# IntelLabs/coach

Measured on AMD Instinct MI355X. Metric: env-steps/sec (+ grad-updates/sec) on Atari-like Clipped-PPO, 64 vectorized envs/GPU, higher is better.
Workload: dtype f32; 1 GPU; C2: Atari-Pong-like Clipped-PPO, 64 vectorized envs/GPU, 84x84x4 uint8 obs, GAE(0.99,0.95), rollout 2048 env-steps (episodes of 32), 10 epochs x 32 minibatches of 64, fp32 conv torso x2 (value/policy), TF1-Adam; parallelism=dp1 (env vectors sharded per GPU, flat fp32 gradient all-reduce), hip_graphs=True

## Files before the change

### coach_amd/_rlx.py

```python
import ctypes
import os
import re
import subprocess
import threading

_HERE = os.path.dirname(os.path.abspath(__file__))
_ROOT = os.path.dirname(_HERE)
HEADER = os.path.join(_ROOT, "include", "rlx.h")
LIB_PATH = os.path.join(_HERE, "librlx.so")
CSRC = os.path.join(_HERE, "csrc")


class RlxUnavailable(RuntimeError):
    """librlx.so is missing or cannot be loaded; the HIP hot path cannot run."""


class RlxError(RuntimeError):
    """A librlx entry point returned a non-zero rlx_status."""


_CTYPE = {
    "int": ctypes.c_int,
    "unsigned": ctypes.c_uint,
    "unsigned int": ctypes.c_uint,
# ... 245 lines not shown

class SplitkJob(STRUCTS["rlx_splitk_job"]):
    __doc__ = STRUCTS["rlx_splitk_job"].__doc__

    def workspace_floats(self):
        return (self.M * self.N + self.N) * self.batch * self.splits if self.splits > 1 else 0


ABI_VERSION = CONSTANTS["RLX_ABI_VERSION"]
NOISY_PASSES = CONSTANTS["RLX_NOISY_PASSES"]
NOISY_MAX_LAYERS = CONSTANTS["RLX_NOISY_MAX_LAYERS"]
NOISY_PASS = {"act": 0, "online": 1, "target": 2, "online_next": 3}
assert sorted(NOISY_PASS.values()) == list(range(NOISY_PASSES)), "NOISY_PASS names every pass of RLX_NOISY_PASSES"
ADAM_TICKET_WORDS = CONSTANTS["RLX_ADAM_TICKET_WORDS"]
MAX_SPLITK_JOBS = CONSTANTS["RLX_MAX_SPLITK_JOBS"]
MAX_COLUMNS = CONSTANTS["RLX_MAX_COLUMNS"]
ACT = {None: CONSTANTS["RLX_ACT_NONE"]}
ACT.update((k[len("RLX_ACT_"):].lower(), v) for k, v in CONSTANTS.items() if k.startswith("RLX_ACT_"))


def make_columns(pairs):
    arr = (Column * len(pairs))()
    for i, (s, d) in enumerate(pairs):
        rb = (s[0].numel() if s.dim() > 1 else 1) * s.element_size()
        arr[i] = Column(s.data_ptr(), d.data_ptr(), rb)
    return arr


def splitk_reduce_jobs(jobs, stream=None, ppo_tail=None, per_tail=None):
    live = [j for j in jobs if j.splits > 1]
    s = current_stream() if stream is None else stream
    for i in range(0, len(live), MAX_SPLITK_JOBS):
        chunk = live[i:i + MAX_SPLITK_JOBS]
        arr = (SplitkJob * len(chunk))(*chunk)
        if per_tail is not None and ppo_tail is None and i + MAX_SPLITK_JOBS >= len(live):
            run = lambda a=arr, n=len(chunk), t=per_tail: lib().splitk_reduce_jobs_per_update(ctypes.byref(a), n, *t, s)
            per_tail = None
        elif ppo_tail is not None and i + MAX_SPLITK_JOBS >= len(live):
            run = lambda a=arr, n=len(chunk), t=ppo_tail: lib().splitk_reduce_jobs_ppo_tail(ctypes.byref(a), n, ctypes.byref(t), s)
            ppo_tail = None
        else:
            run = lambda a=arr, n=len(chunk): lib().splitk_reduce_jobs(ctypes.byref(a), n, s)
        _record((), run, flops=0.0)
        run()
    if ppo_tail is not None:
        lib().ppo_heads_tail(ctypes.byref(ppo_tail), s)
    if per_tail is not None:
        lib().per_update(*per_tail, s)


def conv_input_grad(dz, weights, dx, x_out, deriv, tables, B, H, W, C, KH, KW, S, Co, towers, dy_stride, w_stride,
                    dx_stride, stream=None):
    s = current_stream() if stream is None else stream
    OH, OW = (H - KH) // S + 1, (W - KW) // S + 1
    run = lambda: lib().conv_input_grad(dz, weights, dx, x_out, ACT[deriv], tables, B, H, W, C, KH, KW, S, Co, towers,
                                        dy_stride, w_stride, dx_stride, s)
    if GEMM_HOOK is not None:
        d = GemmDesc()
        d.M, d.N, d.K, d.batch = B * OH * OW, KH * KW * C, Co, towers
        _record((d,), run)
    run()


def per_update_desc(args):
    sum_t, min_t, max_t, cap, idx, err, n, alpha, eps, maxp, status = args
    d = PerUpdateDesc()
    d.sum_tree, d.min_tree, d.max_tree, d.capacity = sum_t.data_ptr(), min_t.data_ptr(), max_t.data_ptr(), int(cap)
    d.idx, d.td_errors, d.n, d.alpha, d.epsilon = idx.data_ptr(), err.data_ptr(), int(n), float(alpha), float(eps)
    d.max_priority, d.status = maxp.data_ptr(), status.data_ptr()
    return d


def conv_dw_item(x, x_tower_stride, x_is_u8, a_div, dz, dz_tower_stride, B, H, W, C, KH, KW, S, Co, towers, dw, dw_tower_stride, db,
                 db_tower_stride, workspace):
    it = ConvDwItem()
    it.x, it.x_tower_stride, it.x_is_u8, it.a_div = x.data_ptr(), x_tower_stride, int(bool(x_is_u8)), float(a_div)
    it.dz, it.dz_tower_stride = dz.data_ptr(), dz_tower_stride
    it.B, it.H, it.W, it.C, it.KH, it.KW, it.S, it.filters, it.towers = B, H, W, C, KH, KW, S, Co, towers
    it.dw, it.dw_tower_stride, it.db, it.db_tower_stride = dw.data_ptr(), dw_tower_stride, _ptr(db), db_tower_stride
    it.workspace, it.workspace_floats = workspace.data_ptr(), workspace.numel()
    return it


def conv_dw_multi(items, jobs, stream=None):
    s = current_stream() if stream is None else stream
    n = len(items)
    arr = (ConvDwItem * n)(*items)
    jarr = (SplitkJob * n)()

    def run():
        lib().conv_dw_multi(arr, jarr, n, s)
    if GEMM_HOOK is not None:
        descs = []
        for it in items:
            OH, OW = (it.H - it.KH) // it.S + 1, (it.W - it.KW) // it.S + 1
            d = GemmDesc()
            d.M, d.K = it.KH * it.KW * it.C, it.B * OH * OW
            d.N, d.batch, d.a_is_u8 = (it.towers * it.filters, 1, 1) if it.x_is_u8 else (it.filters, it.towers, 0)
            descs.append(d)
        _record(tuple(descs), run)
    run()
    for j, out in zip(jarr, jobs):
        ctypes.memmove(ctypes.byref(out), ctypes.byref(j), ctypes.sizeof(SplitkJob))


GEMM_HOOK = None
CALL_COUNT = 0


def _ptr(t):
    return None if t is None else (t.data_ptr() if hasattr(t, "data_ptr") else t)


def gemm(M, N, K, A, B, C, *, a_strides=None, a_tabs=None, a_u8=False, a_div=1.0,
         a_vec_along_k=1, a_tab_vec_ok=0, b_strides=None, ldc=None, bias=None, activation=None,
         deriv_aux=None, aux_ld=None, deriv_kind=None, accumulate=False, batch=1,
         a_batch_stride=0, b_batch_stride=0, c_batch_stride=0, bias_batch_stride=0,
         aux_batch_stride=0, workspace=None, colsum_out=None, colsum_batch_stride=0, stream=None,
         batch_inner=0, a_batch_stride2=0, b_batch_stride2=0, bias_batch_stride2=0, n_fold=0, launch=True,
         defer=None, row_heads=None, kw_min_tiles=0):
    d = GemmDesc()
    d.M, d.N, d.K, d.batch = int(M), int(N), int(K), int(batch)
    d.A, d.B, d.C = _ptr(A), _ptr(B), _ptr(C)
    if a_tabs is not None:
        d.a_row_tab, d.a_k_tab = _ptr(a_tabs[0]), _ptr(a_tabs[1])
        d.a_row_stride, d.a_k_stride = 0, 0
    else:
        rs, ks = a_strides if a_strides is not None else (K, 1)
        d.a_row_stride, d.a_k_stride = int(rs), int(ks)
    ks, ns = b_strides if b_strides is not None else (N, 1)
    d.b_k_stride, d.b_n_stride = int(ks), int(ns)
    d.a_batch_stride, d.b_batch_stride = int(a_batch_stride), int(b_batch_stride)
    d.ldc = int(N if ldc is None else ldc)
    d.c_batch_stride, d.bias_batch_stride = int(c_batch_stride), int(bias_batch_stride)
    d.bias, d.deriv_aux = _ptr(bias), _ptr(deriv_aux)
    d.aux_ld = int(N if aux_ld is None else aux_ld)
    d.aux_batch_stride = int(aux_batch_stride)
    d.workspace = _ptr(workspace)
    d.colsum_out, d.colsum_batch_stride = _ptr(colsum_out), int(colsum_batch_stride)
    d.workspace_floats = int(workspace.numel()) if workspace is not None else 0
    d.a_is_u8, d.a_div = int(bool(a_u8)), float(a_div)
    d.a_vec_along_k, d.a_tab_vec_ok = int(a_vec_along_k), int(a_tab_vec_ok)
    d.activation, d.deriv_kind = ACT[activation], ACT[deriv_kind]
    d.accumulate = int(bool(accumulate))
    d.batch_inner = int(batch_inner)
    d.a_batch_stride2, d.b_batch_stride2 = int(a_batch_stride2), int(b_batch_stride2)
    d.bias_batch_stride2 = int(bias_batch_stride2)
    d.n_fold = int(n_fold)
    d.kw_min_tiles = int(kw_min_tiles)
    if row_heads is not None:
        d._row_heads = row_heads
        d.row_heads, d.n_row_heads = ctypes.addressof(row_heads), len(row_heads)
    if not launch:
        return d
    s = current_stream() if stream is None else stream
    if defer is not None:
        run = lambda: lib().gemm_defer(ctypes.byref(d), ctypes.byref(defer), s)
    else:
        run = lambda: lib().gemm(ctypes.byref(d), s)
    _record((d,), run)
    run()


def _record(descs, run, flops=None):
    if GEMM_HOOK is not None:
        GEMM_HOOK({"descs": tuple(GemmDesc.from_buffer_copy(x) for x in descs), "run": run, "flops": flops})


def gemm_pair_or_single(desc, stream=None):
    s = current_stream() if stream is None else stream
    run = lambda: lib().gemm(ctypes.byref(desc), s)
    _record((desc,), run)
    run()

# ... 24 lines not shown
```

### coach_amd/agents/clipped_ppo_agent.py

```python
import os
import random

import numpy as np
import torch

from .. import _rlx
from ..core_types import EnvironmentSteps, RunPhase
from ..memories.episodic.episodic_rollout_buffer import DeviceEpisodicRolloutBuffer
from ..nn.networks import ClippedPPONet
from ..schedules import ConstantSchedule


from ..architectures.scheme_views import SchemeViews


class ClippedPPONetworkParameters(SchemeViews):
    def __init__(self):
        self.activation_function = 'tanh'
        self.embedder_scheme = 'Medium'
        self.middleware_scheme = 'Medium'
        self.batch_size = 64
        self.optimizer_type = 'Adam'
        self.learning_rate = 0.00025
        self.adam_optimizer_beta1 = 0.9
# ... 418 lines not shown
            if self.dist is None:
                mem.gather_next_states(rows, n, self.ds_obs_raw[:n])
                self.norm.push(self.ds_obs_raw[:n])

        def chunk_obs(c0, m):
            if self.norm is not None:
                return self.ds_obs[c0:c0 + m]
            return mem.gather_states(rows[c0:c0 + m], m, self.chunk_obs[:m])
        for c0 in range(0, 0 if recorded else n, self.chunk):
            m = min(self.chunk, n - c0)
            net.values(chunk_obs(c0, m), m, out=self.ds_value[c0:c0 + m])
        n_seq = 1 if self.ragged else mem.n_env
        self.lib.gae(self.ds_reward, self.ds_value, self.ds_done, None, n_seq, n // n_seq,
                     alg.discount, alg.gae_lambda, self.ds_adv64, self.ds_vtarget, s)
        self.lib.standardize(self.ds_adv64, n, self.ds_adv, None, self.adv_stats, s)
        for c0 in range(0, 0 if recorded else n_train, self.chunk):
            m = min(self.chunk, n_train - c0)
            if self.continuous:
                net.policy_mean_std(chunk_obs(c0, m), m, use_target=True, tag="old",
                                    out_mean=self.ds_old_probs[c0:c0 + m], out_std=self.ds_old_std[c0:c0 + m])
            else:
                net.policy_probs(chunk_obs(c0, m), m, use_target=True, tag="old",
                                 out=self.ds_old_probs[c0:c0 + m])

    def fill_advantages(self):
        n = self.memory.num_transitions()
        rows = self.memory.dataset_rows()
        if self.norm is not None and self.dist is not None:
            self.memory.gather_states(rows, n, self.ds_obs_raw[:n])
            self.norm.push_shared(self.ds_obs_raw[:n], self.dist)
        n_train = min(n, self.ap.algorithm.num_consecutive_playing_steps.num_steps)
        recorded = self._records_acting() and not self._rec_missing
        self._run(("fill", n, n_train, recorded), lambda: self._fill_advantages_device(n, rows, n_train, recorded))
        if self.norm is not None and self.dist is not None:
            self.memory.gather_next_states(rows, n, self.ds_obs_raw[:n])
            self.norm.push_shared(self.ds_obs_raw[:n], self.dist)

    def _gather_minibatch(self, m, i=0):
        mem, s = self.memory, _rlx.current_stream()
        rows_all = mem.dataset_rows()
        B = self.ap.network_wrappers["main"].batch_size
        idx, rows = self.perm_dev[i * B:i * B + m], self.mb_rows[:m]
        cols = [(rows_all, rows), (self.ds_action, self.mb_action), (self.ds_adv, self.mb_adv), (self.ds_vtarget, self.mb_vtarget),
                (self.ds_old_probs, self.mb_old)]
        if self.continuous:
            cols.append((self.ds_old_std, self.mb_old_std))
        if self.norm is not None:
            cols.append((self.ds_obs, self.mb_obs))
        self.lib.copy_columns(_rlx.make_columns(cols), len(cols), idx, None, 0, 0, self.ds_adv.numel(), m, m,
                              mem.status, s)
        if self.norm is not None:
            return self.mb_obs[:m]
        return mem.gather_states(rows, m, self.mb_obs[:m])

    def _gather_epoch(self, n):
        mem, s = self.memory, _rlx.current_stream()
        e = self._epoch_buffers()
        cols = [(mem.dataset_rows(), e["rows"]), (self.ds_action, e["action"]), (self.ds_adv, e["adv"]),
                (self.ds_vtarget, e["vtarget"]), (self.ds_old_probs, e["old"])]
        if self.continuous:
            cols.append((self.ds_old_std, e["old_std"]))
        if self.norm is not None:
            cols.append((self.ds_obs, e["obs"]))
        self.lib.copy_columns(_rlx.make_columns(cols), len(cols), self.perm_dev[:n], None, 0, 0, self.ds_adv.numel(), n, n,
                              mem.status, s)
        if self.norm is None:
            mem.gather_states(e["rows"][:n], n, e["obs"][:n])
        return e

    def _epoch_buffers(self):
        e = getattr(self, "_epoch_bufs", None)
        if e is None:
            cap, dev, f32 = self.memory.cap, self.device, torch.float32
            e = self._epoch_bufs = dict(
                rows=torch.empty(cap, dtype=torch.int32, device=dev),
                action=torch.empty((cap, self.A) if self.continuous else (cap,), dtype=self.actions.dtype, device=dev),
                adv=torch.empty(cap, dtype=f32, device=dev), vtarget=torch.empty(cap, dtype=f32, device=dev),
                old=torch.empty(cap, self.A, dtype=f32, device=dev),
                old_std=torch.empty(cap, self.A, dtype=f32, device=dev) if self.continuous else None,
                obs=torch.empty((cap,) + tuple(self.mb_obs.shape[1:]), dtype=self.mb_obs.dtype, device=dev))
        return e

    def _minibatch_fb(self, m, clip_rescaler, stop_after_dense=False, i=0, epoch=None):
        if epoch is not None:
            B = self.ap.network_wrappers["main"].batch_size
            sl = slice(i * B, i * B + m)
            old = (epoch["old"][sl], epoch["old_std"][sl]) if self.continuous else epoch["old"][sl]
            self.networks["main"].forward_backward(epoch["obs"][sl], m, epoch["action"][sl], epoch["adv"][sl],
                                                   epoch["vtarget"][sl], old, clip_rescaler, self.mb_ratio,
                                                   self.mb_clipped, stop_after_dense=stop_after_dense)
            return
        obs = self._gather_minibatch(m, i)
        old = (self.mb_old, self.mb_old_std) if self.continuous else self.mb_old
        self.networks["main"].forward_backward(obs, m, self.mb_action, self.mb_adv, self.mb_vtarget,
                                               old, clip_rescaler, self.mb_ratio, self.mb_clipped,
                                               stop_after_dense=stop_after_dense)

    def _minibatch_finish(self, scale):
        net = self.networks["main"]
        net.finish_update(scale, signal_acc=self.scalar_acc)

    OVERLAP_EDGE_PAIR_US = 50.0

    def _decide_overlap(self, n, clip):
        net, d = self.networks["main"], self.dist
        off = net.late_gradient_offset()
        rec = {"graph_resident": bool(self.use_graphs and d.capturable()), "edge_pair_us": self.OVERLAP_EDGE_PAIR_US,
               "late_bucket_allreduce_us": None, "conv_backward_us": None}
        if not rec["graph_resident"] or off <= 0:
            rec.update(overlap=False, why="collectives are not graph nodes on this backend" if off > 0
                       else "no early-finished bucket (no convolution layers)")
        else:
            B = self.ap.network_wrappers["main"].batch_size
            m = min(B, n)
            e = self._gather_epoch(n)
            ev = [torch.cuda.Event(enable_timing=True) for _ in range(2)]
            us = []
            for _ in range(3):
                self._minibatch_fb(m, clip, True, i=0, epoch=e)
                ev[0].record()
                net.backward_rest()
                ev[1].record()
                ev[1].synchronize()
                us.append(1e3 * ev[0].elapsed_time(ev[1]))
            bw = d.max_over_ranks(min(us))
            ar = d.max_over_ranks(d.all_reduce_us(net.params.grads.numel() - off) or 0.0)
            hidden = min(ar, bw)
            rec.update(late_bucket_allreduce_us=round(ar, 1), conv_backward_us=round(bw, 1), overlap=bool(hidden > self.OVERLAP_EDGE_PAIR_US),
                       why="min(all-reduce, convolution backward) = %.1f us %s the %.0f us edge pair"
                           % (hidden, ">" if hidden > self.OVERLAP_EDGE_PAIR_US else "<=", self.OVERLAP_EDGE_PAIR_US))
        self.overlap_decision = rec
        self.overlap_allreduce = rec["overlap"]

    def train_network(self, order, epochs):
        alg = self.ap.algorithm
        netp = self.ap.network_wrappers["main"]
        B = netp.batch_size
        n = len(order)
        self.networks["main"].set_clip_rescaler(float(alg.clipping_decay_schedule.current_value))
        clip = None
        scale = self.dist.grad_scale(netp.scale_down_gradients_by_number_of_workers_for_sync_training) \
            if self.dist else 1.0
        results = []
        for j in range(epochs):
            batch_order = list(range(n))
            random.shuffle(batch_order)
            order = [order[i] for i in batch_order]
            full = np.zeros(self.perm_dev.numel(), dtype=np.int32)
            full[:n] = order
            self._perm.push(full)
            self.scalar_acc.zero_()
            nmb = -(-n // B)
            if self.overlap_allreduce is None:
                self._decide_overlap(n, clip)
            in_graph = self.dist is not None and self.use_graphs and self.dist.capturable()
            net = self.networks["main"]

            def reduced_fb(m, i, e=None):
                if self.overlap_allreduce and net.late_gradient_offset() > 0:
                    grads, off = net.params.grads, net.late_gradient_offset()
                    self._minibatch_fb(m, clip, True, i=i, epoch=e)
                    w1 = self.dist.all_reduce_sum_async(grads[off:])
                    net.backward_rest()
                    w2 = self.dist.all_reduce_sum_async(grads[:off])
                    w1.wait()
                    w2.wait()
                else:
                    self._minibatch_fb(m, clip, i=i, epoch=e)
                    self.dist.all_reduce_sum(net.params.grads)

            if (self.dist is None or in_graph) and self.epoch_graph and not self.ragged:
                def epoch():
                    e = self._gather_epoch(n)
                    for i in range(nmb):
                        if self.dist is None:
                            self._minibatch_fb(min(B, n - i * B), clip, i=i, epoch=e)
                        else:
                            reduced_fb(min(B, n - i * B), i, e)
                        self._minibatch_finish(scale)
# ... 73 lines not shown
```

### coach_amd/csrc/conv_dw_multi.hip

```cpp
#include "conv_dw_body.hpp"

namespace {

using namespace rlx_convdw;

struct MultiArgs {
    DwU8 u8;
    DwF32 f[2];
    int nb_u8, nb_f[2], kind[2];
    int u8_half;
};

template <int PASSES>
__global__ void __launch_bounds__(kThreads) conv_dw_multi_kernel(const MultiArgs m) {
    extern __shared__ __attribute__((aligned(16))) float smem[];
    int bid = blockIdx.x;
    if (bid < m.nb_u8) {
        if (m.u8_half) conv_dw_u8_body_half(m.u8, bid, smem);
        else if constexpr (PASSES > 1) conv_dw_u8_body_passes<PASSES>(m.u8, bid, smem);
        else conv_dw_u8_body<20, 16, 84>(m.u8, bid, smem);
        return;
    }
    bid -= m.nb_u8;
#pragma unroll
    for (int i = 0; i < 2; ++i) {
        if (bid < m.nb_f[i]) {
            if (m.kind[i] == 1) {
                if constexpr (PASSES > 1) conv_dw_f32_body_two_pass<64, 3, 1, 9, 7, 4, 7>(m.f[i], bid, smem);
                else conv_dw_f32_body<64, 3, 1, 9, 7>(m.f[i], bid, smem);
            } else {
                if constexpr (PASSES > 1) conv_dw_f32_body_two_pass<32, 4, 2, 20, 9, 5, 9>(m.f[i], bid, smem);
                else conv_dw_f32_body<32, 4, 2, 20, 9>(m.f[i], bid, smem);
            }
            return;
        }
        bid -= m.nb_f[i];
    }
}

int g_passes = 2;
int g_pairs_per_wg = 0;
inline int pairs_per_wg(int B, int towers) {
    if (g_passes <= 1) return 1;
    if (g_pairs_per_wg > 0) return g_pairs_per_wg;
    return towers * ((B + 1) / 2) >= 64 ? 2 : 1;
}

}

extern "C" {

int rlx_conv_dw_multi(const rlx_conv_dw_item *items, rlx_splitk_job *jobs, int n_items, void *stream) {
    RLX_REQUIRE(items && jobs && n_items >= 1 && n_items <= 3, "rlx_conv_dw_multi: 1 .. 3 items");
    int n_u8 = 0, n_f = 0;
    bool one = n_items >= 2;
    GeometryU8 gu;
    GeometryF32 gf[2];
    const rlx_conv_dw_item *iu = nullptr, *fi[2] = {nullptr, nullptr};
    int ju = -1, jf[2] = {-1, -1};
    for (int i = 0; i < n_items && one; ++i) {
        const rlx_conv_dw_item &it = items[i];
        if (it.x_is_u8) {
            one = n_u8 == 0 && geometry_u8(it.B, it.H, it.W, it.C, it.KH, it.KW, it.S, it.filters, it.towers, &gu) && gu.OW == 20 &&
                  gu.OH == 20 && it.S * it.C == 16 && gu.rowf == 336;
            iu = &it; ju = i; ++n_u8;
        } else {
            one = n_f < 2 && geometry_f32(it.B, it.H, it.W, it.C, it.KH, it.KW, it.S, it.filters, it.towers, &gf[n_f < 2 ? n_f : 1],
                                          pairs_per_wg(it.B, it.towers));
            if (n_f < 2) { fi[n_f] = &it; jf[n_f] = i; }
            ++n_f;
        }
    }
    if (!one) {
        for (int i = 0; i < n_items; ++i) {
            const rlx_conv_dw_item &it = items[i];
            const int rc = it.x_is_u8
                ? rlx_conv_dw_u8(static_cast<const unsigned char *>(it.x), it.a_div, it.dz, it.dz_tower_stride, it.B, it.H, it.W, it.C,
                                 it.KH, it.KW, it.S, it.filters, it.towers, it.dw, it.dw_tower_stride, it.db, it.db_tower_stride,
                                 it.workspace, it.workspace_floats, &jobs[i], stream)
                : rlx_conv_dw_f32(static_cast<const float *>(it.x), it.x_tower_stride, it.dz, it.dz_tower_stride, it.B, it.H, it.W,
                                  it.C, it.KH, it.KW, it.S, it.filters, it.towers, it.dw, it.dw_tower_stride, it.db,
                                  it.db_tower_stride, it.workspace, it.workspace_floats, &jobs[i], stream);
            if (rc != RLX_OK) return rc;
        }
        return RLX_OK;
    }
    MultiArgs m;
    m.nb_u8 = m.nb_f[0] = m.nb_f[1] = 0;
    m.kind[0] = m.kind[1] = 0;
    m.u8_half = 0;
    size_t lds = 0;
    if (iu) {
        const rlx_conv_dw_item &it = *iu;
        RLX_REQUIRE(it.x && it.dz && it.dw && it.workspace && it.a_div != 0.f, "rlx_conv_dw_multi: null pointer (uint8 item)");
        const long long need = (long long)it.B * ((long long)gu.K * kN + kN);
        RLX_REQUIRE(it.workspace_floats >= need, "rlx_conv_dw_multi: workspace of %lld floats, need %lld", it.workspace_floats, need);
        RLX_REQUIRE((((uintptr_t)it.x) & 3) == 0 && ((((uintptr_t)it.dz) | ((uintptr_t)it.workspace)) & 15) == 0 &&
                        (it.dz_tower_stride & 3) == 0, "rlx_conv_dw_multi: misaligned operand (uint8 item)");
        DwU8 &a = m.u8;
        a.x = static_cast<const unsigned char *>(it.x); a.dz = it.dz; a.dz_ts = it.dz_tower_stride;
        a.part = it.workspace; a.cpart = it.workspace + (size_t)it.B * gu.K * kN;
        a.a_div = it.a_div;
        a.B = it.B; a.H = it.H; a.W = it.W; a.C = it.C; a.KH = it.KH; a.S = it.S; a.OH = gu.OH; a.OW = gu.OW; a.Co = it.filters;
        a.K = gu.K; a.P = gu.P; a.rowf = gu.rowf; a.NQ = gu.NQ; a.stamps = nullptr;
        m.nb_u8 = ((it.B + 7) / 8) * 8 * gu.NQ;
        m.u8_half = gu.nch == kNH;
        lds = gu.lds;
        rlx_splitk_job &j = jobs[ju];
        j.partials = a.part; j.colsum_partials = it.db ? a.cpart : nullptr;
        j.C = it.dw; j.colsum_out = it.db;
        j.ldc = it.filters; j.c_batch_stride = it.dw_tower_stride; j.colsum_batch_stride = it.db_tower_stride;
        j.M = gu.K; j.N = gu.nch; j.batch = 1; j.splits = gu.splits; j.n_fold = it.filters;
    }
    for (int k = 0; k < 2; ++k) {
        if (!fi[k]) continue;
        const rlx_conv_dw_item &it = *fi[k];
        const GeometryF32 &g = gf[k];
        RLX_REQUIRE(it.x && it.dz && it.dw && it.workspace, "rlx_conv_dw_multi: null pointer (fp32 item)");
        const long long need = (long long)it.towers * g.splits * ((long long)g.K * kN + kN);
        RLX_REQUIRE(it.workspace_floats >= need, "rlx_conv_dw_multi: workspace of %lld floats, need %lld", it.workspace_floats, need);
        RLX_REQUIRE(((((uintptr_t)it.x) | ((uintptr_t)it.dz) | ((uintptr_t)it.workspace)) & 15) == 0 && (it.x_tower_stride & 3) == 0 &&
                        (it.dz_tower_stride & 3) == 0, "rlx_conv_dw_multi: misaligned operand (fp32 item)");
        DwF32 &a = m.f[k];
        a.x = static_cast<const float *>(it.x); a.x_ts = it.x_tower_stride; a.dz = it.dz; a.dz_ts = it.dz_tower_stride;
        a.part = it.workspace; a.cpart = it.db ? it.workspace + (size_t)it.towers * g.splits * g.K * kN : nullptr;
        a.B = it.B; a.H = it.H; a.OH = g.OH; a.KH = it.KH; a.splits = g.splits; a.units = it.towers * g.splits;
        a.ppw = pairs_per_wg(it.B, it.towers);
        a.stamps = nullptr;
        m.nb_f[k] = ((a.units + 7) / 8) * 8 * it.KH;
        m.kind[k] = g.kind;
        lds = g.lds > lds ? g.lds : lds;
        rlx_splitk_job &j = jobs[jf[k]];
        j.partials = a.part; j.colsum_partials = a.cpart;
        j.C = it.dw; j.colsum_out = it.db;
        j.ldc = it.filters; j.c_batch_stride = it.dw_tower_stride; j.colsum_batch_stride = it.db_tower_stride;
        j.M = g.K; j.N = kN; j.batch = it.towers; j.splits = g.splits; j.n_fold = 0;
    }
    static bool configured = false;
    if (!configured) {
        RLX_HIP(hipFuncSetAttribute(reinterpret_cast<const void *>(conv_dw_multi_kernel<1>),
                                    hipFuncAttributeMaxDynamicSharedMemorySize, 160 * 1024));
        RLX_HIP(hipFuncSetAttribute(reinterpret_cast<const void *>(conv_dw_multi_kernel<2>),
                                    hipFuncAttributeMaxDynamicSharedMemorySize, 160 * 1024));
        RLX_HIP(hipFuncSetAttribute(reinterpret_cast<const void *>(conv_dw_multi_kernel<4>),
                                    hipFuncAttributeMaxDynamicSharedMemorySize, 160 * 1024));
        configured = true;
    }
    const unsigned grid = m.nb_u8 + m.nb_f[0] + m.nb_f[1];
    if (g_passes > 1) {
        size_t lds2 = iu ? (m.u8_half ? lds_u8_half() : (g_passes == 4 ? lds_u8_passes<4>() : lds_u8_passes<2>())) : 0;
        for (int k = 0; k < 2; ++k) {
            if (!fi[k]) continue;
            const size_t l = m.kind[k] == 2 ? lds_f32_two_pass<32, 20, 9, 5>() : lds_f32_two_pass<64, 9, 7, 4>();
            lds2 = l > lds2 ? l : lds2;
        }
        if (g_passes == 4) RLX_LAUNCH((conv_dw_multi_kernel<4>), grid, kThreads, lds2, rlx::as_stream(stream), m);
        else RLX_LAUNCH((conv_dw_multi_kernel<2>), grid, kThreads, lds2, rlx::as_stream(stream), m);
    } else {
        RLX_LAUNCH((conv_dw_multi_kernel<1>), grid, kThreads, lds, rlx::as_stream(stream), m);
    }
    RLX_LAUNCH_CHECK();
    return RLX_OK;
}

int rlx_conv_dw_pairs_per_workgroup(int pairs) {
    RLX_REQUIRE(pairs >= 0 && pairs <= 2, "rlx_conv_dw_pairs_per_workgroup: 0 (by the number of workgroups), 1 or 2");
    g_pairs_per_wg = pairs;
    return RLX_OK;
}

int rlx_conv_dw_passes(int passes) {
    RLX_REQUIRE(passes == 1 || passes == 2 || passes == 4, "rlx_conv_dw_passes: 1, 2 or 4");
    g_passes = passes;
    return RLX_OK;
}

}
```

### coach_amd/csrc/gemm.hip

```cpp
#include "rlx_common.hpp"
#include "dense_small_body.hpp"
#include "losses_body.hpp"
#include "splitk_reduce_body.hpp"
#include <cstdlib>

namespace {

typedef float f32x16 __attribute__((ext_vector_type(16)));
typedef float f32x4 __attribute__((ext_vector_type(4)));

constexpr int BK = 32;
constexpr int kThreads = 256;
constexpr int kTabChunk = 2048;
constexpr int kWinChunk = 1024;

struct OperandDev {
    const void *base;
    const int *tab_o;
    const int *tab_r;
    long long stride_o, stride_r, batch_stride, batch_stride2;
    int vec_ok;
};

struct GemmDev {
    int xcd_mode;
    OperandDev a, b;
    float *c;
    long long ldc, c_batch_stride;
    const float *bias;
    long long bias_batch_stride, bias_batch_stride2;
    int inner;
    const float *aux;
    long long aux_ld, aux_batch_stride;
    float *ws;
    float *colsum;
    float *ws_colsum;
    long long colsum_batch_stride;
    int M, N, K;
    int splits, kchunk;
    int act, deriv, accumulate;
    int vec_epi;
    int fold;
    float a_div;
    unsigned long long *stamps;
    const int *win_row_yx;
    const int *win_k_jyx;
    const int *win_b_koff;
    const int *win_c_row;
    int win_oh, win_ow;
    int win_rows_per_phase;
};

__device__ __forceinline__ long long batch_off(int batch, int inner, long long stride, long long stride2) {
    const int bo = batch / inner;
    return (long long)bo * stride2 + (long long)(batch - bo * inner) * stride;
}

__device__ __forceinline__ float apply_act(float v, int act) {
    if (act == RLX_ACT_RELU) return v > 0.f ? v : 0.f;
    if (act == RLX_ACT_TANH) return tanhf(v);
    return v;
}
__device__ __forceinline__ float act_deriv(float y, int kind) {
    if (kind == RLX_ACT_RELU) return y > 0.f ? 1.f : 0.f;
    if (kind == RLX_ACT_TANH) return 1.f - y * y;
    return 1.f;
}

template <bool VEC_RED, bool U8>
__device__ __forceinline__ float4 load4(const OperandDev &op, const unsigned char *base, int o,
                                        int r, int o_lim, int r_lim, float div) {
    float4 v = make_float4(0.f, 0.f, 0.f, 0.f);
    if (o >= o_lim || r >= r_lim) return v;
    const long long off_o = op.tab_o ? (long long)op.tab_o[o] : (long long)o * op.stride_o;
    const long long off_r = op.tab_r ? (long long)op.tab_r[r] : (long long)r * op.stride_r;
    const int remaining = VEC_RED ? (r_lim - r) : (o_lim - o);
    if (op.vec_ok && remaining >= 4) {
        if (U8) {
            const uint32_t w = *reinterpret_cast<const uint32_t *>(base + off_o + off_r);
            v.x = (float)(w & 0xffu) / div;
            v.y = (float)((w >> 8) & 0xffu) / div;
            v.z = (float)((w >> 16) & 0xffu) / div;
            v.w = (float)(w >> 24) / div;
        } else {
            v = *reinterpret_cast<const float4 *>(reinterpret_cast<const float *>(base) + off_o + off_r);
// ... 1544 lines not shown
            const int k = wave * kq + lane + 64 * j;
            if (k < k1) {
                const float xv = hrow[k];
#pragma unroll
                for (int n = 0; n < NN; ++n)
                    if (n < hp.N) acc[n] = fmaf(xv, wreg[j][n], acc[n]);
            }
        }
#pragma unroll
        for (int n = 0; n < NN; ++n) {
            float v = acc[n];
#pragma unroll
            for (int o = 32; o > 0; o >>= 1) v += __shfl_xor(v, o, 64);
            if (lane == 0) hpart[wave][n] = v;
        }
    }
    __syncthreads();
    if ((int)threadIdx.x < hp.N) {
        const int n = threadIdx.x;
        float v = ((hpart[0][n] + hpart[1][n]) + hpart[2][n]) + hpart[3][n];
        v += hp.b ? hp.b[n] : 0.f;
        v = rlx_small::act_apply(v, hp.act);
        hp.y[(size_t)row * hp.N + n] = v;
        if (PPO) yrow[n] = v;
    }
    if (!PPO) return;
    const int kind = r.kind[batch];
    if (kind == 0) return;
    if (kind == 2) {
        const int tid = threadIdx.x;
        if (tid < hp.N) porow[tid] = pre;
        else if (tid == 16) prow[0] = pre;
        else if (tid == 17) prow_act = pre_i;
        else if (tid == 18) prow[1] = pre;
    }
    __syncthreads();
    if (wave == 0) {
        using namespace rlx_losses;
        const int B = g.M;
        if (kind == 1) {
            if (lane == 0) {
                const float w = 1.f;
                const float e = yrow[0] - pre;
                float l, gg;
                regression_terms(e, 0, l, gg);
                dzrow[0] = regression_grad(r.grad_scale, w, gg, B);
                r.row_terms[(size_t)row * 4] = w * l;
                if (r.dy[batch]) r.dy[batch][row] = dzrow[0];
            }
        } else {
            PpoRowTerms t;
            float *dyr = r.dy[batch] ? r.dy[batch] + (size_t)row * hp.N : nullptr;
            if (!ppo_discrete_row_wave(yrow, porow, prow_act, hp.N, prow[0], prow[1], r.beta, r.grad_scale, B, dzrow,
                                       r.ratio_out ? r.ratio_out + row : nullptr, r.clipped_out ? r.clipped_out + row : nullptr, t)) {
                if (lane == 0) atomicOr(r.status, 1);
                if (lane < hp.N) dzrow[lane] = 0.f;
                t.sur = t.ent = t.kl = 0.f;
            }
            if (lane == 0) {
                r.row_terms[(size_t)row * 4 + 1] = t.sur;
                r.row_terms[(size_t)row * 4 + 2] = t.ent;
                r.row_terms[(size_t)row * 4 + 3] = t.kl;
            }
            if (dyr && lane < hp.N) dyr[lane] = dzrow[lane];
        }
    }
    __syncthreads();
    if (wave < 4 && r.dx[batch]) {
        float *dx = r.dx[batch] + (size_t)row * hp.K;
#pragma unroll
        for (int j = 0; j < P; ++j) {
            const int k = wave * kq + lane + 64 * j;
            if (k < k1) {
                float s = 0.f;
#pragma unroll
                for (int n = 0; n < NN; ++n)
                    if (n < hp.N) s = fmaf(dzrow[n], wreg[j][n], s);
                dx[k] = r.lower_act ? s * rlx_small::act_deriv_out(hrow[k], r.lower_act) : s;
            }
        }
    }
}

struct PpoTailDev {
    rlx_small::SmallDenseBwd value, policy;
    const float *row_terms;
    float *scalars;
    int batch, red_threads, nn;
    float beta;
};
template <int NN>
__device__ __forceinline__ void ppo_heads_tail_body(const PpoTailDev &a, int kblock, bool is_policy, float *smem,
                                                    float (*red)[256]) {
    using namespace rlx_losses;
    const rlx_small::SmallDenseBwd &p = is_policy ? a.policy : a.value;
    if (kblock * rlx_small::kKL >= p.K) return;
    if (kblock == 0) {
        const int b = threadIdx.x, B = a.batch;
        if (is_policy) {
            float l_sur = 0.f, l_ent = 0.f, l_kl = 0.f;
            if (b < B) {
                l_sur = a.row_terms[(size_t)b * 4 + 1];
                l_ent = a.row_terms[(size_t)b * 4 + 2];
                l_kl = a.row_terms[(size_t)b * 4 + 3];
            }
            block_sum3_first(l_sur, l_ent, l_kl, red, a.red_threads);
            if (threadIdx.x == 0) ppo_discrete_scalars(l_sur, l_ent, l_kl, a.beta, B, a.scalars);
        } else {
            const float local = b < B ? a.row_terms[(size_t)b * 4] : 0.f;
            const float s = block_sum_first(local, red[0], a.red_threads);
            if (threadIdx.x == 0) a.scalars[4] = s / (float)B;
        }
    }
    rlx_small::dense_small_bwd_body<NN, rlx_small::kKL, rlx_small::kRG, false>(p, kblock, 0, smem);
}
constexpr int kTailSmemFloats = 256 * rlx_small::kMaxN + rlx_small::kRG * rlx_small::kKL * rlx_small::kMaxN;

template <int NN>
__global__ void __launch_bounds__(256) ppo_heads_tail_kernel(const PpoTailDev a) {
    __shared__ float smem[kTailSmemFloats];
    __shared__ float red[3][256];
    ppo_heads_tail_body<NN>(a, blockIdx.x, blockIdx.z == 1, smem, red);
}

using rlx_reduce::ReduceJobs;
using rlx_reduce::splitk_reduce_job_body;
__global__ void __launch_bounds__(1024) splitk_reduce_jobs_kernel(const ReduceJobs jobs) {
    __shared__ float4 part[16][64];
    splitk_reduce_job_body(jobs.job[blockIdx.z], part);
}
template <int NN>
__global__ void __launch_bounds__(1024) splitk_reduce_jobs_tail_kernel(const ReduceJobs jobs, int n_jobs, const PpoTailDev tail) {
    __shared__ float4 part[16][64];
    __shared__ float smem[kTailSmemFloats];
    __shared__ float red[3][256];
    if (blockIdx.z > 0) {
        splitk_reduce_job_body(jobs.job[blockIdx.z - 1], part);
        return;
    }
    if (blockIdx.y > 1 || threadIdx.x >= 256) return;
    ppo_heads_tail_body<NN>(tail, blockIdx.x, blockIdx.y == 1, smem, red);
}

__global__ void colsum_partial_kernel(const float *__restrict__ x, int M, int N, long long ld,
                                      int rows_per_block, float *__restrict__ part) {
    const int n = blockIdx.x * blockDim.x + threadIdx.x;
    if (n >= N) return;
    const int r0 = blockIdx.y * rows_per_block, r1 = min(M, r0 + rows_per_block);
    float s = 0.f;
    for (int r = r0; r < r1; ++r) s += x[(size_t)r * ld + n];
    part[(size_t)blockIdx.y * N + n] = s;
}
__global__ void colsum_final_kernel(const float *__restrict__ part, int nparts, int N,
                                    float *__restrict__ out, int accumulate) {
    const int n = blockIdx.x * blockDim.x + threadIdx.x;
    if (n >= N) return;
    float s = 0.f;
    for (int p = 0; p < nparts; ++p) s += part[(size_t)p * N + n];
    out[n] = accumulate ? out[n] + s : s;
}

__global__ void act_backward_kernel(float *__restrict__ dy, const float *__restrict__ y, long long n,
                                    int kind) {
    for (long long i = (long long)blockIdx.x * blockDim.x + threadIdx.x; i < n;
         i += (long long)gridDim.x * blockDim.x)
        dy[i] *= act_deriv(y[i], kind);
}

__global__ void conv_tables_kernel(int *__restrict__ rowbase, int *__restrict__ koff, int batch,
                                   int H, int W, int C, int KH, int KW, int stride, int OH, int OW) {
    const int t = blockIdx.x * blockDim.x + threadIdx.x;
    const int M = batch * OH * OW, K = KH * KW * C;
    if (t < M) {
        const int ox = t % OW, oy = (t / OW) % OH, b = t / (OW * OH);
        rowbase[t] = ((b * H + oy * stride) * W + ox * stride) * C;
    }
    if (t < K) {
        const int c = t % C, kx = (t / C) % KW, ky = t / (C * KW);
        koff[t] = (ky * W + kx) * C + c;
    }
}

__global__ void conv_dx_tables_kernel(int *__restrict__ rowbase, int *__restrict__ yx, int *__restrict__ crow,
                                      int *__restrict__ koff_a, int *__restrict__ jyx, int *__restrict__ koff_b,
                                      int batch, int H, int W, int C, int KH, int KW, int s, int Co, int OH, int OW,
                                      int Mp) {
    const int t = blockIdx.x * blockDim.x + threadIdx.x;
    const int P = s * s, Hq = (H + s - 1) / s, Wq = (W + s - 1) / s, Jx = KW / s, K = (KH / s) * Jx * Co;
    if (t < P * Mp) {
        const int ph = t / Mp, r = t - ph * Mp, py = ph / s, px = ph - py * s;
        const int X = r % Wq, Y = (r / Wq) % Hq, b = r / (Wq * Hq);
        const int iy = s * Y + py, ix = s * X + px;
        const bool real = r < batch * Hq * Wq && iy < H && ix < W;
        rowbase[t] = real ? ((b * OH + Y) * OW + X) * Co : 0;
        yx[t] = real ? (Y << 16) | X : (0x7fff << 16);
        crow[t] = real ? ((b * H + iy) * W + ix) * C : -1;
    }
    if (t < K) {
        const int tap = t / Co, co = t - tap * Co, jy = tap / Jx, jx = tap - jy * Jx;
// ... 533 lines not shown
        RLX_REQUIRE(BM * BN == 4096, "rlx_gemm: internal tile selection error");
        rc = narrow ? launch_variant<128, 32>(g, a_vec_red, d.a_is_u8 != 0, b_vec_red, grid, s)
                    : launch_variant<64, 64>(g, a_vec_red, d.a_is_u8 != 0, b_vec_red, grid, s);
    }
    RLX_REQUIRE(rc == 0, "rlx_gemm: unsupported operand combination (uint8 A with transposed B)");
    RLX_LAUNCH_CHECK();
    if (splits > 1) {
        if (defer && deferrable(g, d.M, d.N)) {
            fill_job(defer, g, d.M, d.N, d.batch, splits);
            return RLX_OK;
        }
        if (d.row_heads && d.n_row_heads > 0 && launch_reduce_with_row_heads(g, d, splits, s)) {
            tl_row_heads_done = true;
            RLX_LAUNCH_CHECK();
            return RLX_OK;
        }
        return launch_splitk_reduce(g, d.M, d.N, d.batch, splits, s);
    }
    return RLX_OK;
}

}

extern "C" {

int rlx_gemm_describe(const rlx_gemm_desc *desc, int *out8_host) {
    RLX_REQUIRE(desc && out8_host, "rlx_gemm_describe: null pointer");
    GemmPlan plan{};
    const int rc = gemm_impl(desc, nullptr, &plan, nullptr);
    if (rc != RLX_OK) return rc;
    out8_host[0] = plan.q_fast; out8_host[1] = plan.q_bm; out8_host[2] = plan.q_bn; out8_host[3] = plan.q_kw;
    out8_host[4] = plan.q_splits; out8_host[5] = plan.q_kchunk; out8_host[6] = plan.q_ring; out8_host[7] = plan.thin;
    return RLX_OK;
}

int rlx_gemm(const rlx_gemm_desc *d_host, void *stream) {
    tl_row_heads_done = false;
    const int rc = gemm_impl(d_host, stream, nullptr);
    if (rc != RLX_OK || !d_host->row_heads || d_host->n_row_heads <= 0 || tl_row_heads_done) return rc;
    return rlx_dense_small_forward_multi(d_host->row_heads, d_host->n_row_heads, stream);
}

static int gemm_pair_impl(const rlx_gemm_desc *weight_grad, const rlx_gemm_desc *input_grad, void *stream,
                          rlx_splitk_job *defer);

int rlx_gemm_pair(const rlx_gemm_desc *weight_grad, const rlx_gemm_desc *input_grad, void *stream) {
    return gemm_pair_impl(weight_grad, input_grad, stream, nullptr);
}

int rlx_gemm_defer(const rlx_gemm_desc *desc_host, rlx_splitk_job *job_host, void *stream) {
    RLX_REQUIRE(job_host != nullptr, "rlx_gemm_defer: null job");
    return gemm_impl(desc_host, stream, nullptr, job_host);
}

int rlx_gemm_pair_defer(const rlx_gemm_desc *weight_grad, const rlx_gemm_desc *input_grad,
                        rlx_splitk_job *weight_grad_job_host, void *stream) {
    RLX_REQUIRE(weight_grad_job_host != nullptr, "rlx_gemm_pair_defer: null job");
    return gemm_pair_impl(weight_grad, input_grad, stream, weight_grad_job_host);
}

int rlx_splitk_reduce_jobs(const rlx_splitk_job *jobs_host, int n_jobs, void *stream) {
    RLX_REQUIRE(jobs_host && n_jobs >= 0 && n_jobs <= RLX_MAX_SPLITK_JOBS,
                "rlx_splitk_reduce_jobs: 0..%d jobs (got %d)", RLX_MAX_SPLITK_JOBS, n_jobs);
    ReduceJobs jobs;
    int n = 0, gx = 1, gy = 1;
    for (int i = 0; i < n_jobs; ++i) {
        const rlx_splitk_job &j = jobs_host[i];
        if (j.splits <= 1) continue;
        RLX_REQUIRE(j.partials && j.C && j.M > 0 && j.N > 0 && j.N % 4 == 0 && j.batch > 0 &&
                    (long long)j.M * j.N < (1LL << 31) && aligned16(j.partials),
                    "rlx_splitk_reduce_jobs: job %d is not a float4-reducible product", i);
        jobs.job[n++] = j;
        const int bx = (int)(((long long)j.M * j.N / 4 + 63) / 64);
        gx = bx > gx ? bx : gx;
        gy = j.batch > gy ? j.batch : gy;
    }
    if (n == 0) return RLX_OK;
    RLX_LAUNCH((splitk_reduce_jobs_kernel), dim3(gx, gy, n), 1024, 0, rlx::as_stream(stream), jobs);
    RLX_LAUNCH_CHECK();
    return RLX_OK;
}

namespace {
int ppo_rows_check(const rlx_ppo_rows_desc *q, const char *who) {
    RLX_REQUIRE(q && q->value_targets && q->actions && q->advantages && q->old_probs && q->row_terms && q->scalars &&
                q->status, "%s: null pointer", who);
    const rlx_small_dense_problem *h[2] = {&q->value_head, &q->policy_head};
    for (int i = 0; i < 2; ++i) {
        RLX_REQUIRE(h[i]->x && h[i]->w && h[i]->y && h[i]->dy && h[i]->dw && h[i]->dx, "%s: null pointer in head %d", who, i);
        RLX_REQUIRE(h[i]->towers == 1 && h[i]->M == q->batch && h[i]->K > 0 && h[i]->activation == 0,
                    "%s: head %d must be one linear tower over the %d rows of the batch", who, i, q->batch);
        RLX_REQUIRE(h[i]->lower_activation >= 0 && h[i]->lower_activation <= 2, "%s: unknown activation", who);
    }
    RLX_REQUIRE(q->value_head.N == 1 && q->policy_head.N >= 2 && q->policy_head.N <= rlx_small::kMaxN &&
                q->value_head.K == q->policy_head.K && q->value_head.lower_activation == q->policy_head.lower_activation,
                "%s: value head N = 1, policy head 2 <= N <= %d, both on the same dense layer", who, rlx_small::kMaxN);
    RLX_REQUIRE(q->batch >= 1 && q->batch <= 256, "%s: 1 <= batch <= 256 (one row per thread in the scalar sums)", who);
    return RLX_OK;
}
PpoTailDev ppo_tail_dev(const rlx_ppo_rows_desc &q) {
    PpoTailDev t{};
    const rlx_small_dense_problem *h[2] = {&q.value_head, &q.policy_head};
    rlx_small::SmallDenseBwd *d[2] = {&t.value, &t.policy};
    for (int i = 0; i < 2; ++i)
        *d[i] = rlx_small::SmallDenseBwd{h[i]->x, 0, h[i]->w, 0, h[i]->dy, 0, nullptr, 0, h[i]->dw, 0, h[i]->db, 0, nullptr, 0,
                                         h[i]->M, h[i]->K, h[i]->N, 0, 0};
    t.row_terms = q.row_terms; t.scalars = q.scalars; t.batch = q.batch; t.beta = q.beta_entropy;
    t.red_threads = 64;
    while (t.red_threads < q.batch) t.red_threads <<= 1;
    t.nn = q.policy_head.N <= 4 ? 4 : (q.policy_head.N <= 8 ? 8 : 16);
    return t;
}
}

int rlx_ppo_fc_rows_supported(const rlx_gemm_desc *fc, int n_actions) {
    if (!fc || fc->row_heads || fc->batch != 2 || fc->N % 4 != 0 || fc->N > 1024 || fc->M > 256 || n_actions < 2 ||
        n_actions > rlx_small::kMaxN || fc->ldc != fc->N || fc->n_fold > 0 || fc->colsum_out)
        return 0;
    GemmPlan plan{};
    if (gemm_impl(fc, nullptr, &plan, nullptr) != RLX_OK) return 0;
    return plan.q_splits > 16 ? 1 : 0;
}

int rlx_ppo_fc_rows(const rlx_gemm_desc *fc, const rlx_ppo_rows_desc *rows, void *stream) {
    const int rc0 = ppo_rows_check(rows, "rlx_ppo_fc_rows");
    if (rc0 != RLX_OK) return rc0;
    RLX_REQUIRE(fc && !fc->row_heads && rlx_ppo_fc_rows_supported(fc, rows->policy_head.N) && fc->M == rows->batch &&
                fc->N == rows->value_head.K,
                "rlx_ppo_fc_rows: not a product rlx_ppo_fc_rows_supported accepts, or its shape does not match the heads");
    rlx_small_dense_problem heads[2] = {rows->value_head, rows->policy_head};
    rlx_gemm_desc d = *fc;
    d.row_heads = heads;
    d.n_row_heads = 2;
    tl_row_heads_done = false;
    tl_ppo_rows = rows;
    const int rc = gemm_impl(&d, stream, nullptr);
    tl_ppo_rows = nullptr;
    if (rc != RLX_OK) return rc;
    RLX_REQUIRE(tl_row_heads_done, "rlx_ppo_fc_rows: the product did not take the row-finishing reduction");
    return RLX_OK;
}

int rlx_ppo_heads_tail(const rlx_ppo_rows_desc *rows, void *stream) {
    const int rc0 = ppo_rows_check(rows, "rlx_ppo_heads_tail");
    if (rc0 != RLX_OK) return rc0;
    const PpoTailDev t = ppo_tail_dev(*rows);
    const int kb = (rows->value_head.K + rlx_small::kKL - 1) / rlx_small::kKL;
    dim3 grid(kb, 1, 2);
    hipStream_t s = rlx::as_stream(stream);
    if (t.nn == 4) RLX_LAUNCH((ppo_heads_tail_kernel<4>), grid, 256, 0, s, t);
    else if (t.nn == 8) RLX_LAUNCH((ppo_heads_tail_kernel<8>), grid, 256, 0, s, t);
    else RLX_LAUNCH((ppo_heads_tail_kernel<16>), grid, 256, 0, s, t);
    RLX_LAUNCH_CHECK();
    return RLX_OK;
}

int rlx_splitk_reduce_jobs_ppo_tail(const rlx_splitk_job *jobs_host, int n_jobs, const rlx_ppo_rows_desc *rows, void *stream) {
    RLX_REQUIRE(jobs_host && n_jobs >= 0 && n_jobs <= RLX_MAX_SPLITK_JOBS,
                "rlx_splitk_reduce_jobs_ppo_tail: 0..%d jobs (got %d)", RLX_MAX_SPLITK_JOBS, n_jobs);
    const int rc0 = ppo_rows_check(rows, "rlx_splitk_reduce_jobs_ppo_tail");
    if (rc0 != RLX_OK) return rc0;
    ReduceJobs jobs;
    int n = 0, gx = 1, gy = 1;
    for (int i = 0; i < n_jobs; ++i) {
        const rlx_splitk_job &j = jobs_host[i];
        if (j.splits <= 1) continue;
        RLX_REQUIRE(j.partials && j.C && j.M > 0 && j.N > 0 && j.N % 4 == 0 && j.batch > 0 &&
                    (long long)j.M * j.N < (1LL << 31) && aligned16(j.partials),
                    "rlx_splitk_reduce_jobs_ppo_tail: job %d is not a float4-reducible product", i);
        jobs.job[n++] = j;
        const int bx = (int)(((long long)j.M * j.N / 4 + 63) / 64);
        gx = bx > gx ? bx : gx;
        gy = j.batch > gy ? j.batch : gy;
    }
    if (n == 0) return rlx_ppo_heads_tail(rows, stream);
    const PpoTailDev t = ppo_tail_dev(*rows);
    const int kb = (rows->value_head.K + rlx_small::kKL - 1) / rlx_small::kKL;
    gx = kb > gx ? kb : gx;
    gy = gy < 2 ? 2 : gy;
    dim3 grid(gx, gy, n + 1);
    hipStream_t s = rlx::as_stream(stream);
    if (t.nn == 4) RLX_LAUNCH((splitk_reduce_jobs_tail_kernel<4>), grid, 1024, 0, s, jobs, n, t);
    else if (t.nn == 8) RLX_LAUNCH((splitk_reduce_jobs_tail_kernel<8>), grid, 1024, 0, s, jobs, n, t);
    else RLX_LAUNCH((splitk_reduce_jobs_tail_kernel<16>), grid, 1024, 0, s, jobs, n, t);
    RLX_LAUNCH_CHECK();
    return RLX_OK;
}

static int gemm_pair_impl(const rlx_gemm_desc *weight_grad, const rlx_gemm_desc *input_grad, void *stream,
                          rlx_splitk_job *defer) {
    if (defer) defer->splits = 0;
    GemmPlan pw, px;
    int rc = gemm_impl(weight_grad, stream, &pw);
    if (rc != RLX_OK) return rc;
    rc = gemm_impl(input_grad, stream, &px);
// ... 242 lines not shown
```

### coach_amd/csrc/optim.hip

```cpp
#include "rlx_common.hpp"

namespace {

constexpr int kBlock = 256;

#if defined(__HIP_DEVICE_COMPILE__) && !defined(__gfx950__) && !defined(__gfx942__)
#error "optim.hip: the last-arriver ticket protocol is written for gfx950 (gfx942-compatible) only"
#endif

constexpr unsigned kTicketGroups = 32, kTicketStride = 32;
static_assert(kTicketStride * (1 + kTicketGroups) == RLX_ADAM_TICKET_WORDS, "rlx.h: RLX_ADAM_TICKET_WORDS");
__device__ __forceinline__ bool draw_last_ticket(unsigned int *ticket) {
    const unsigned G = gridDim.x < kTicketGroups ? gridDim.x : kTicketGroups;
    const unsigned grp = blockIdx.x % G, gsize = (gridDim.x - grp + G - 1) / G;
    unsigned int *gw = ticket + kTicketStride * (1 + grp);
    if (__hip_atomic_fetch_add(gw, 1u, __ATOMIC_RELAXED, __HIP_MEMORY_SCOPE_AGENT) != gsize - 1) return false;
    __hip_atomic_store(gw, 0u, __ATOMIC_RELAXED, __HIP_MEMORY_SCOPE_AGENT);
    if (__hip_atomic_fetch_add(ticket, 1u, __ATOMIC_RELAXED, __HIP_MEMORY_SCOPE_AGENT) != G - 1) return false;
    __hip_atomic_store(ticket, 0u, __ATOMIC_RELAXED, __HIP_MEMORY_SCOPE_AGENT);
    return true;
}

template <bool NORM>
__global__ void adam_tf1_kernel(float *__restrict__ w, const float *__restrict__ g,
                                float *__restrict__ m, float *__restrict__ v, long long n,
                                float lr, float beta1, float beta2, float eps,
                                const float *__restrict__ state, float grad_scale,
                                float *__restrict__ sumsq_part) {
    __shared__ float red[kBlock];
    float ss = 0.f;
    const float b1p = state[0], b2p = state[1];
    const float alpha = lr * sqrtf(1.f - b2p) / (1.f - b1p);
    const float omb1 = 1.f - beta1, omb2 = 1.f - beta2;
    const long long stride = (long long)gridDim.x * blockDim.x;
    const long long n4 = n >> 2;
    for (long long i = (long long)blockIdx.x * blockDim.x + threadIdx.x; i < n4; i += stride) {
        float4 gw = reinterpret_cast<const float4 *>(g)[i];
        float4 mw = reinterpret_cast<float4 *>(m)[i];
        float4 vw = reinterpret_cast<float4 *>(v)[i];
        float4 ww = reinterpret_cast<float4 *>(w)[i];
        float *gp = &gw.x, *mp = &mw.x, *vp = &vw.x, *wp = &ww.x;
#pragma unroll
        for (int k = 0; k < 4; ++k) {
            if (NORM) ss += gp[k] * gp[k];
            const float gr = gp[k] * grad_scale;
            mp[k] += (gr - mp[k]) * omb1;
            vp[k] += (gr * gr - vp[k]) * omb2;
            wp[k] -= (mp[k] * alpha) / (sqrtf(vp[k]) + eps);
        }
        reinterpret_cast<float4 *>(m)[i] = mw;
        reinterpret_cast<float4 *>(v)[i] = vw;
        reinterpret_cast<float4 *>(w)[i] = ww;
    }
    for (long long i = (n4 << 2) + (long long)blockIdx.x * blockDim.x + threadIdx.x; i < n; i += stride) {
        if (NORM) ss += g[i] * g[i];
        const float gr = g[i] * grad_scale;
        m[i] += (gr - m[i]) * omb1;
        v[i] += (gr * gr - v[i]) * omb2;
        w[i] -= (m[i] * alpha) / (sqrtf(v[i]) + eps);
    }
    if (NORM) {
        red[threadIdx.x] = ss;
        __syncthreads();
        for (int d = kBlock >> 1; d > 0; d >>= 1) {
            if (threadIdx.x < d) red[threadIdx.x] += red[threadIdx.x + d];
            __syncthreads();
        }
        if (threadIdx.x == 0) sumsq_part[blockIdx.x] = red[0];
    }
}


template <bool NORM, bool MIX, bool TICKET>
__global__ void __launch_bounds__(kBlock)
adam_step_kernel(float *__restrict__ w, const float *__restrict__ g, float *__restrict__ m, float *__restrict__ v,
                 long long n, float lr, float beta1, float beta2, float eps, float *state, float grad_scale,
                 float *sumsq_part, float *__restrict__ target, float rate, float one_minus_rate,
                 unsigned int *ticket, float *norm_out, const float *acc_src, float *acc_dst, int n_acc) {
    __shared__ float red[kBlock];
    __shared__ int last_s;
    float ss = 0.f;
    const float b1p = state[0], b2p = state[1];
    const float alpha = lr * sqrtf(1.f - b2p) / (1.f - b1p);
    const float omb1 = 1.f - beta1, omb2 = 1.f - beta2;
    const long long stride = (long long)gridDim.x * blockDim.x;
    const long long n4 = n >> 2;
    for (long long i = (long long)blockIdx.x * blockDim.x + threadIdx.x; i < n4; i += stride) {
        float4 gw = reinterpret_cast<const float4 *>(g)[i];
        float4 mw = reinterpret_cast<float4 *>(m)[i];
        float4 vw = reinterpret_cast<float4 *>(v)[i];
        float4 ww = reinterpret_cast<float4 *>(w)[i];
        float4 tw = MIX ? reinterpret_cast<float4 *>(target)[i] : make_float4(0.f, 0.f, 0.f, 0.f);
        float *gp = &gw.x, *mp = &mw.x, *vp = &vw.x, *wp = &ww.x, *tp = &tw.x;
#pragma unroll
        for (int k = 0; k < 4; ++k) {
            if (NORM) ss += gp[k] * gp[k];
            const float gr = gp[k] * grad_scale;
            mp[k] += (gr - mp[k]) * omb1;
            vp[k] += (gr * gr - vp[k]) * omb2;
            wp[k] -= (mp[k] * alpha) / (sqrtf(vp[k]) + eps);
            if (MIX) tp[k] = rate * wp[k] + one_minus_rate * tp[k];
        }
        reinterpret_cast<float4 *>(m)[i] = mw;
        reinterpret_cast<float4 *>(v)[i] = vw;
        reinterpret_cast<float4 *>(w)[i] = ww;
        if (MIX) reinterpret_cast<float4 *>(target)[i] = tw;
    }
    for (long long i = (n4 << 2) + (long long)blockIdx.x * blockDim.x + threadIdx.x; i < n; i += stride) {
        if (NORM) ss += g[i] * g[i];
        const float gr = g[i] * grad_scale;
        m[i] += (gr - m[i]) * omb1;
        v[i] += (gr * gr - v[i]) * omb2;
        w[i] -= (m[i] * alpha) / (sqrtf(v[i]) + eps);
        if (MIX) target[i] = rate * w[i] + one_minus_rate * target[i];
    }
    if (NORM) {
        red[threadIdx.x] = ss;
        __syncthreads();
        for (int d = kBlock >> 1; d > 0; d >>= 1) {
            if (threadIdx.x < d) red[threadIdx.x] += red[threadIdx.x + d];
            __syncthreads();
        }
        if (threadIdx.x == 0) {
            if (TICKET) __hip_atomic_store(&sumsq_part[blockIdx.x], red[0], __ATOMIC_RELAXED, __HIP_MEMORY_SCOPE_AGENT);
            else sumsq_part[blockIdx.x] = red[0];
        }
    }
    if (!TICKET) return;
    __syncthreads();
    if (threadIdx.x == 0) {
        if (NORM) asm volatile("s_waitcnt vmcnt(0)" ::: "memory");
        const bool last = draw_last_ticket(ticket);
        if (last && !NORM) {
            state[0] = b1p * beta1;
            state[1] = b2p * beta2;
        }
        last_s = last;
    }
    if (!NORM) return;
    __syncthreads();
    if (!last_s) return;
    __builtin_amdgcn_fence(__ATOMIC_ACQUIRE, "agent");
    float s = 0.f;
    for (int i = threadIdx.x; i < (int)gridDim.x; i += kBlock)
        s += __hip_atomic_load(&sumsq_part[i], __ATOMIC_RELAXED, __HIP_MEMORY_SCOPE_AGENT);
    red[threadIdx.x] = s;
    __syncthreads();
    for (int d = kBlock >> 1; d > 0; d >>= 1) {
        if (threadIdx.x < d) red[threadIdx.x] += red[threadIdx.x + d];
        __syncthreads();
    }
    if (threadIdx.x == 0) {
        norm_out[0] = sqrtf(red[0]);
        state[0] = b1p * beta1;
        state[1] = b2p * beta2;
        for (int i = 0; i < n_acc; ++i) acc_dst[i] += acc_src[i];
    }
}

constexpr int kNormIt = 4;
template <bool MIX>
__global__ void __launch_bounds__(kBlock)
adam_step_norm_kernel(float *__restrict__ w, const float *__restrict__ g, float *__restrict__ m, float *__restrict__ v,
                      long long n, float lr, float beta1, float beta2, float eps, float *state, float grad_scale,
                      float *sumsq_part, float *__restrict__ target, float rate, float one_minus_rate,
                      unsigned int *ticket, float *norm_out, const float *acc_src, float *acc_dst, int n_acc) {
    __shared__ float red[kBlock];
    __shared__ int last_s;
    const float b1p = state[0], b2p = state[1];
    const float alpha = lr * sqrtf(1.f - b2p) / (1.f - b1p);
    const float omb1 = 1.f - beta1, omb2 = 1.f - beta2;
    const long long stride = (long long)gridDim.x * blockDim.x;
    const long long n4 = n >> 2;
    const long long i0 = (long long)blockIdx.x * blockDim.x + threadIdx.x;
    float4 gw[kNormIt], mw[kNormIt], vw[kNormIt], ww[kNormIt], tw[kNormIt];
#pragma unroll
    for (int it = 0; it < kNormIt; ++it) {
        const long long i = i0 + it * stride;
        if (i < n4) {
            gw[it] = reinterpret_cast<const float4 *>(g)[i];
            mw[it] = reinterpret_cast<float4 *>(m)[i];
            vw[it] = reinterpret_cast<float4 *>(v)[i];
            ww[it] = reinterpret_cast<float4 *>(w)[i];
            if (MIX) tw[it] = reinterpret_cast<float4 *>(target)[i];
        }
    }
    const long long it0 = (n4 << 2) + i0;
    const bool has_tail = it0 < n;
    const float gt = has_tail ? g[it0] : 0.f;
    float ss = 0.f;
#pragma unroll
    for (int it = 0; it < kNormIt; ++it)
        if (i0 + it * stride < n4) {
            const float *gp = &gw[it].x;
#pragma unroll
            for (int k = 0; k < 4; ++k) ss += gp[k] * gp[k];
        }
    if (has_tail) ss += gt * gt;
    red[threadIdx.x] = ss;
    __syncthreads();
    for (int d = kBlock >> 1; d > 0; d >>= 1) {
        if (threadIdx.x < d) red[threadIdx.x] += red[threadIdx.x + d];
        __syncthreads();
    }
    float old = 0.f;
    if (threadIdx.x == 0)
        old = __hip_atomic_exchange(&sumsq_part[blockIdx.x], red[0], __ATOMIC_RELAXED, __HIP_MEMORY_SCOPE_AGENT);
#pragma unroll
    for (int it = 0; it < kNormIt; ++it) {
        const long long i = i0 + it * stride;
        if (i < n4) {
            float *gp = &gw[it].x, *mp = &mw[it].x, *vp = &vw[it].x, *wp = &ww[it].x, *tp = &tw[it].x;
#pragma unroll
            for (int k = 0; k < 4; ++k) {
                const float gr = gp[k] * grad_scale;
                mp[k] += (gr - mp[k]) * omb1;
                vp[k] += (gr * gr - vp[k]) * omb2;
                wp[k] -= (mp[k] * alpha) / (sqrtf(vp[k]) + eps);
                if (MIX) tp[k] = rate * wp[k] + one_minus_rate * tp[k];
            }
            reinterpret_cast<float4 *>(m)[i] = mw[it];
            reinterpret_cast<float4 *>(v)[i] = vw[it];
            reinterpret_cast<float4 *>(w)[i] = ww[it];
            if (MIX) reinterpret_cast<float4 *>(target)[i] = tw[it];
        }
    }
    if (has_tail) {
        const float gr = gt * grad_scale;
        m[it0] += (gr - m[it0]) * omb1;
        v[it0] += (gr * gr - v[it0]) * omb2;
        w[it0] -= (m[it0] * alpha) / (sqrtf(v[it0]) + eps);
        if (MIX) target[it0] = rate * w[it0] + one_minus_rate * target[it0];
    }
    if (threadIdx.x == 0) {
        asm volatile("" ::"v"(old) : "memory");
        last_s = draw_last_ticket(ticket);
    }
    __syncthreads();
    if (!last_s) return;
    __builtin_amdgcn_fence(__ATOMIC_ACQUIRE, "agent");
    float s = 0.f;
    for (int i = threadIdx.x; i < (int)gridDim.x; i += kBlock)
        s += __hip_atomic_load(&sumsq_part[i], __ATOMIC_RELAXED, __HIP_MEMORY_SCOPE_AGENT);
    red[threadIdx.x] = s;
    __syncthreads();
    for (int d = kBlock >> 1; d > 0; d >>= 1) {
        if (threadIdx.x < d) red[threadIdx.x] += red[threadIdx.x + d];
        __syncthreads();
    }
    if (threadIdx.x == 0) {
        norm_out[0] = sqrtf(red[0]);
        state[0] = b1p * beta1;
        state[1] = b2p * beta2;
        for (int i = 0; i < n_acc; ++i) acc_dst[i] += acc_src[i];
    }
}

__global__ void adam_advance_kernel(float *state, float beta1, float beta2) {
    state[0] *= beta1;
    state[1] *= beta2;
}

__global__ void adam_finish_norm_kernel(float *state, float beta1, float beta2,
                                        const float *__restrict__ part, int nparts,
                                        float *__restrict__ norm_out, const float *acc_src,
                                        float *acc_dst, int n_acc) {
    __shared__ float red[kBlock];
    float s = 0.f;
    for (int i = threadIdx.x; i < nparts; i += kBlock) s += part[i];
    red[threadIdx.x] = s;
    __syncthreads();
    for (int d = kBlock >> 1; d > 0; d >>= 1) {
        if (threadIdx.x < d) red[threadIdx.x] += red[threadIdx.x + d];
        __syncthreads();
    }
    if (threadIdx.x == 0) {
        norm_out[0] = sqrtf(red[0]);
        state[0] *= beta1;
        state[1] *= beta2;
        for (int i = 0; i < n_acc; ++i) acc_dst[i] += acc_src[i];
    }
}

__global__ void mix_kernel(float *__restrict__ target, const float *__restrict__ online, long long n,
                           float rate, float one_minus_rate) {
    const long long stride = (long long)gridDim.x * blockDim.x;
    const long long n4 = n >> 2;
    for (long long i = (long long)blockIdx.x * blockDim.x + threadIdx.x; i < n4; i += stride) {
        const float4 o = reinterpret_cast<const float4 *>(online)[i];
        float4 t = reinterpret_cast<float4 *>(target)[i];
        t.x = rate * o.x + one_minus_rate * t.x;
        t.y = rate * o.y + one_minus_rate * t.y;
        t.z = rate * o.z + one_minus_rate * t.z;
        t.w = rate * o.w + one_minus_rate * t.w;
        reinterpret_cast<float4 *>(target)[i] = t;
    }
    for (long long i = (n4 << 2) + (long long)blockIdx.x * blockDim.x + threadIdx.x; i < n; i += stride)
        target[i] = rate * online[i] + one_minus_rate * target[i];
}

__global__ void sumsq_partial_kernel(const float *__restrict__ x, long long n, float *__restrict__ part) {
    __shared__ float red[kBlock];
    float s = 0.f;
    for (long long i = (long long)blockIdx.x * blockDim.x + threadIdx.x; i < n;
         i += (long long)gridDim.x * blockDim.x)
        s += x[i] * x[i];
    red[threadIdx.x] = s;
    __syncthreads();
    for (int d = kBlock >> 1; d > 0; d >>= 1) {
        if (threadIdx.x < d) red[threadIdx.x] += red[threadIdx.x + d];
        __syncthreads();
    }
    if (threadIdx.x == 0) part[blockIdx.x] = red[0];
}
__global__ void sumsq_final_kernel(const float *__restrict__ part, int nparts, float *__restrict__ out) {
    __shared__ float red[kBlock];
    float s = 0.f;
    for (int i = threadIdx.x; i < nparts; i += kBlock) s += part[i];
    red[threadIdx.x] = s;
    __syncthreads();
    for (int d = kBlock >> 1; d > 0; d >>= 1) {
        if (threadIdx.x < d) red[threadIdx.x] += red[threadIdx.x + d];
        __syncthreads();
    }
    if (threadIdx.x == 0) out[0] = sqrtf(red[0]);
}

__global__ void clip_by_global_norm_kernel(float *__restrict__ g, long long n, const float *__restrict__ norm,
                                           float clip) {
    const float inv_norm = 1.0f / *norm, inv_clip = 1.0f / clip;
    const float scale = clip * (inv_clip < inv_norm ? inv_clip : inv_norm);
    const long long stride = (long long)gridDim.x * blockDim.x;
    for (long long i = (long long)blockIdx.x * blockDim.x + threadIdx.x; i < n; i += stride) g[i] *= scale;
}

__global__ void clip_by_value_kernel(float *__restrict__ g, long long n, float clip) {
    const long long stride = (long long)gridDim.x * blockDim.x;
    for (long long i = (long long)blockIdx.x * blockDim.x + threadIdx.x; i < n; i += stride) {
        float x = g[i];
        x = x < -clip ? -clip : x;
        g[i] = x > clip ? clip : x;
    }
}

int g_norm_in_kernel = 2;
}

extern "C" {

int rlx_adam_init(float *m, float *v, long long n, float *state, float beta1, float beta2,
                  void *stream) {
    RLX_REQUIRE(m && v && state && n > 0, "rlx_adam_init: bad arguments");
    hipStream_t s = rlx::as_stream(stream);
    RLX_HIP(hipMemsetAsync(m, 0, sizeof(float) * n, s));
    RLX_HIP(hipMemsetAsync(v, 0, sizeof(float) * n, s));
    const float init[2] = {beta1, beta2};
    RLX_HIP(hipMemcpyAsync(state, init, sizeof(init), hipMemcpyHostToDevice, s));
    return RLX_OK;
}

int rlx_adam_tf1(float *weights, const float *grads, float *m, float *v, long long n,
                 float learning_rate, float beta1, float beta2, float epsilon, float *state,
                 float grad_scale, void *stream) {
    RLX_REQUIRE(weights && grads && m && v && state, "rlx_adam_tf1: null pointer");
    RLX_REQUIRE(n > 0, "rlx_adam_tf1: empty parameter buffer");
    RLX_REQUIRE((((uintptr_t)weights | (uintptr_t)grads | (uintptr_t)m | (uintptr_t)v) & 15) == 0,
                "rlx_adam_tf1: buffers must be 16-byte aligned");
    hipStream_t s = rlx::as_stream(stream);
    RLX_LAUNCH((adam_tf1_kernel<false>), rlx::grid_for(n / 4 + 1, kBlock), kBlock, 0, s, weights, grads, m, v, n, learning_rate, beta1, beta2, epsilon, state, grad_scale, nullptr);
    RLX_LAUNCH_CHECK();
    RLX_LAUNCH((adam_advance_kernel), 1, 1, 0, s, state, beta1, beta2);
    RLX_LAUNCH_CHECK();
    return RLX_OK;
}

int rlx_adam_tf1_norm(float *weights, const float *grads, float *m, float *v, long long n,
                      float learning_rate, float beta1, float beta2, float epsilon, float *state,
                      float grad_scale, float *norm_out, float *workspace, long long workspace_floats,
                      const float *acc_src, float *acc_dst, int n_acc, void *stream) {
    RLX_REQUIRE(weights && grads && m && v && state && norm_out && workspace,
                "rlx_adam_tf1_norm: null pointer");
    RLX_REQUIRE(n > 0, "rlx_adam_tf1_norm: empty parameter buffer");
    RLX_REQUIRE(n_acc == 0 || (acc_src && acc_dst && n_acc > 0 && n_acc <= 64),
                "rlx_adam_tf1_norm: bad signal accumulation arguments");
    RLX_REQUIRE((((uintptr_t)weights | (uintptr_t)grads | (uintptr_t)m | (uintptr_t)v) & 15) == 0,
                "rlx_adam_tf1_norm: buffers must be 16-byte aligned");
    int blocks = rlx::grid_for(n / 4 + 1, kBlock, 1024);
    if (blocks > workspace_floats) blocks = (int)workspace_floats;
    RLX_REQUIRE(blocks >= 1, "rlx_adam_tf1_norm: workspace too small");
    hipStream_t s = rlx::as_stream(stream);
    RLX_LAUNCH((adam_tf1_kernel<true>), blocks, kBlock, 0, s, weights, grads, m, v, n, learning_rate, beta1, beta2,
                                                    epsilon, state, grad_scale, workspace);
    RLX_LAUNCH_CHECK();
    RLX_LAUNCH((adam_finish_norm_kernel), 1, kBlock, 0, s, state, beta1, beta2, workspace, blocks, norm_out, acc_src,
                                                 acc_dst, n_acc);
    RLX_LAUNCH_CHECK();
    return RLX_OK;
}

int rlx_adam_norm_in_kernel(int on) {
    g_norm_in_kernel = on;
    return RLX_OK;
}

int rlx_adam_tf1_step(float *weights, const float *grads, float *m, float *v, long long n, float learning_rate,
                      float beta1, float beta2, float epsilon, float *state, float grad_scale, float *norm_out,
                      float *workspace, long long workspace_floats, const float *acc_src, float *acc_dst, int n_acc,
                      float *target, double mix_rate, unsigned int *ticket, void *stream) {
    RLX_REQUIRE(weights && grads && m && v && state && ticket, "rlx_adam_tf1_step: null pointer");
    RLX_REQUIRE(n > 0, "rlx_adam_tf1_step: empty parameter buffer");
    RLX_REQUIRE(!norm_out || workspace, "rlx_adam_tf1_step: the gradient norm needs a workspace");
    RLX_REQUIRE(n_acc == 0 || (acc_src && acc_dst && n_acc > 0 && n_acc <= 64),
                "rlx_adam_tf1_step: bad signal accumulation arguments");
    RLX_REQUIRE((((uintptr_t)weights | (uintptr_t)grads | (uintptr_t)m | (uintptr_t)v | (uintptr_t)target) & 15) == 0,
                "rlx_adam_tf1_step: buffers must be 16-byte aligned");
    int blocks = rlx::grid_for(n / 4 + 1, kBlock, 1024);
    if (norm_out && blocks > workspace_floats) blocks = (int)workspace_floats;
    RLX_REQUIRE(blocks >= 1, "rlx_adam_tf1_step: workspace too small");
    hipStream_t s = rlx::as_stream(stream);
    const float rate = (float)mix_rate, omr = (float)(1.0 - mix_rate);
#define RLX_ADAM_STEP(NORM, MIX, TICKET)                                                                      \
    RLX_LAUNCH((adam_step_kernel<NORM, MIX, TICKET>), blocks, kBlock, 0, s, weights, grads, m, v, n, learning_rate, beta1,  \
                                                                  beta2, epsilon, state, grad_scale, workspace, \
                                                                  target, rate, omr, ticket, nullptr, nullptr, nullptr, 0)
    if (norm_out && g_norm_in_kernel == 2 && (n >> 2) <= (long long)blocks * kBlock * kNormIt) {
        if (target)
            RLX_LAUNCH((adam_step_norm_kernel<true>), blocks, kBlock, 0, s, weights, grads, m, v, n, learning_rate, beta1, beta2,
                       epsilon, state, grad_scale, workspace, target, rate, omr, ticket, norm_out, acc_src, acc_dst, n_acc);
        else
            RLX_LAUNCH((adam_step_norm_kernel<false>), blocks, kBlock, 0, s, weights, grads, m, v, n, learning_rate, beta1, beta2,
                       epsilon, state, grad_scale, workspace, target, rate, omr, ticket, norm_out, acc_src, acc_dst, n_acc);
        RLX_LAUNCH_CHECK();
        return RLX_OK;
    }
    if (norm_out && g_norm_in_kernel == 1) {
        if (target)
            RLX_LAUNCH((adam_step_kernel<true, true, true>), blocks, kBlock, 0, s, weights, grads, m, v, n, learning_rate, beta1,
                       beta2, epsilon, state, grad_scale, workspace, target, rate, omr, ticket, norm_out, acc_src, acc_dst, n_acc);
        else
            RLX_LAUNCH((adam_step_kernel<true, false, true>), blocks, kBlock, 0, s, weights, grads, m, v, n, learning_rate, beta1,
                       beta2, epsilon, state, grad_scale, workspace, target, rate, omr, ticket, norm_out, acc_src, acc_dst, n_acc);
        RLX_LAUNCH_CHECK();
        return RLX_OK;
    }
    if (norm_out && target) RLX_ADAM_STEP(true, true, false);
    else if (norm_out) RLX_ADAM_STEP(true, false, false);
    else if (target) RLX_ADAM_STEP(false, true, true);
    else RLX_ADAM_STEP(false, false, true);
#undef RLX_ADAM_STEP
    RLX_LAUNCH_CHECK();
    if (norm_out) {
        RLX_LAUNCH((adam_finish_norm_kernel), 1, kBlock, 0, s, state, beta1, beta2, workspace, blocks, norm_out, acc_src,
                                                     acc_dst, n_acc);
        RLX_LAUNCH_CHECK();
    } else if (n_acc > 0) {
        RLX_REQUIRE(false, "rlx_adam_tf1_step: signal sums ride with the norm finish (give norm_out)");
    }
    return RLX_OK;
}

int rlx_mix_weights(float *target, const float *online, long long n, double rate, void *stream) {
    RLX_REQUIRE(target && online && n > 0, "rlx_mix_weights: bad arguments");
    RLX_REQUIRE((((uintptr_t)target | (uintptr_t)online) & 15) == 0,
                "rlx_mix_weights: buffers must be 16-byte aligned");
    RLX_LAUNCH((mix_kernel), rlx::grid_for(n / 4 + 1, kBlock), kBlock, 0, rlx::as_stream(stream), target, online, n, (float)rate, (float)(1.0 - rate));
    RLX_LAUNCH_CHECK();
    return RLX_OK;
}

int rlx_global_norm(const float *x, long long n, float *norm_out, float *workspace,
                    long long workspace_floats, void *stream) {
    RLX_REQUIRE(x && norm_out && workspace && n > 0, "rlx_global_norm: bad arguments");
    int parts = rlx::grid_for(n, kBlock, 1024);
    if (parts > workspace_floats) parts = (int)workspace_floats;
    RLX_REQUIRE(parts >= 1, "rlx_global_norm: workspace too small");
    hipStream_t s = rlx::as_stream(stream);
    RLX_LAUNCH((sumsq_partial_kernel), parts, kBlock, 0, s, x, n, workspace);
    RLX_LAUNCH_CHECK();
    RLX_LAUNCH((sumsq_final_kernel), 1, kBlock, 0, s, workspace, parts, norm_out);
    RLX_LAUNCH_CHECK();
    return RLX_OK;
}

int rlx_clip_by_global_norm(float *grads, long long n, const float *global_norm, float clip_norm,
                            void *stream) {
    RLX_REQUIRE(grads && global_norm && n > 0, "rlx_clip_by_global_norm: bad arguments");
    RLX_REQUIRE(clip_norm > 0.f, "rlx_clip_by_global_norm: clip_norm must be positive (got %g)", (double)clip_norm);
    RLX_LAUNCH((clip_by_global_norm_kernel), rlx::grid_for(n, kBlock, 1024), kBlock, 0, rlx::as_stream(stream), grads, n, global_norm, clip_norm);
    RLX_LAUNCH_CHECK();
    return RLX_OK;
}

int rlx_clip_by_value(float *grads, long long n, float clip_value, void *stream) {
    RLX_REQUIRE(grads && n > 0, "rlx_clip_by_value: bad arguments");
    RLX_REQUIRE(clip_value > 0.f, "rlx_clip_by_value: clip_value must be positive (got %g)", (double)clip_value);
    RLX_LAUNCH((clip_by_value_kernel), rlx::grid_for(n, kBlock, 1024), kBlock, 0, rlx::as_stream(stream), grads, n, clip_value);
    RLX_LAUNCH_CHECK();
    return RLX_OK;
}

}
```

### coach_amd/csrc/splitk_reduce_body.hpp

```cpp
#pragma once
#include "rlx_common.hpp"

namespace rlx_reduce {

struct ReduceJobs {
    rlx_splitk_job job[RLX_MAX_SPLITK_JOBS];
};
__device__ __forceinline__ void splitk_reduce_job_body(const rlx_splitk_job &g, float4 (*part)[64]) {
    constexpr int SG = 16;
    const int batch = blockIdx.y;
    if (batch >= g.batch) return;
    const int mn4 = (g.M * g.N) >> 2;
    if ((int)blockIdx.x * 64 >= mn4 && !(blockIdx.x == 0 && g.colsum_out)) return;
    const int ox = threadIdx.x & 63, q = threadIdx.x >> 6;
    const int gid = blockIdx.x * 64 + ox;
    const size_t mn = (size_t)g.M * g.N;
    const float4 *ws = reinterpret_cast<const float4 *>(g.partials + (size_t)batch * g.splits * mn);
    float4 s = make_float4(0.f, 0.f, 0.f, 0.f);
    if (gid < mn4) {
        int k = q;
        for (; k + 3 * SG < g.splits; k += 4 * SG) {
            const float4 a = ws[(size_t)k * mn4 + gid];
            const float4 b = ws[(size_t)(k + SG) * mn4 + gid];
            const float4 c = ws[(size_t)(k + 2 * SG) * mn4 + gid];
            const float4 d = ws[(size_t)(k + 3 * SG) * mn4 + gid];
            s.x += a.x; s.y += a.y; s.z += a.z; s.w += a.w;
            s.x += b.x; s.y += b.y; s.z += b.z; s.w += b.w;
            s.x += c.x; s.y += c.y; s.z += c.z; s.w += c.w;
            s.x += d.x; s.y += d.y; s.z += d.z; s.w += d.w;
        }
        for (; k < g.splits; k += SG) {
            const float4 a = ws[(size_t)k * mn4 + gid];
            s.x += a.x; s.y += a.y; s.z += a.z; s.w += a.w;
        }
    }
    part[q][ox] = s;
    __syncthreads();
    if (q == 0 && gid < mn4) {
        float v[4] = {s.x, s.y, s.z, s.w};
#pragma unroll
        for (int t = 1; t < SG; ++t) {
            const float4 p = part[t][ox];
            v[0] += p.x; v[1] += p.y; v[2] += p.z; v[3] += p.w;
        }
        const int i = gid << 2;
        const int row = i / g.N, col = i - row * g.N;
        const int tw = g.n_fold ? col / g.n_fold : batch, cl = g.n_fold ? col % g.n_fold : col;
        float *c = g.C + (size_t)tw * g.c_batch_stride + (size_t)row * g.ldc + cl;
        if ((g.ldc & 3) == 0 && (((uintptr_t)c) & 15) == 0) {
            *reinterpret_cast<float4 *>(c) = make_float4(v[0], v[1], v[2], v[3]);
        } else {
            c[0] = v[0]; c[1] = v[1]; c[2] = v[2]; c[3] = v[3];
        }
    }
    if (g.colsum_out && blockIdx.x == 0) {
        float *cpart = reinterpret_cast<float *>(&part[0][0]);
        for (int n0 = 0; n0 < g.N; n0 += 64) {
            __syncthreads();
            const int n = n0 + ox;
            float t = 0.f;
            if (n < g.N)
                for (int k = q; k < g.splits; k += SG)
                    t += g.colsum_partials[((size_t)batch * g.splits + k) * g.N + n];
            cpart[q * 64 + ox] = t;
            __syncthreads();
            if (q == 0 && n < g.N) {
#pragma unroll
                for (int u = 1; u < SG; ++u) t += cpart[u * 64 + ox];
                if (g.n_fold)
                    g.colsum_out[(size_t)(n / g.n_fold) * g.colsum_batch_stride + n % g.n_fold] = t;
                else
                    g.colsum_out[(size_t)batch * g.colsum_batch_stride + n] = t;
            }
        }
    }
}

}
```

### coach_amd/nn/graph.py

```python
import ctypes
import math
import os

import numpy as np
import torch

from .. import _rlx

ALIGN = 4
SMALL_N = 16
FOLD_SHARED_INPUT = True


def _thin_takes(M, N, K, batch):
    return K <= 1024 and N * K <= (1 << 18) and -(-M // 64) * -(-N // 64) * batch <= 96


def _fold(M, N, K, T):
    return FOLD_SHARED_INPUT and not (_thin_takes(M, N, K, T) and K >= 64)


def _align(n):
    return (n + ALIGN - 1) // ALIGN * ALIGN

# ... 28 lines not shown
        n = int(np.prod(shape))
        return buf[off + tower * stride: off + tower * stride + n].view(*shape)

    def w(self, name, tower=0, buf=None):
        return self.view(self.weights if buf is None else buf, name, tower)

    def g(self, name, tower=0):
        return self.view(self.grads, name, tower)

    def stride(self, name):
        return self.entries[name][3]

    def named_arrays(self, buf=None):
        out = {}
        for name, (off, shape, towers, stride) in self.entries.items():
            out[name] = [self.view(self.weights if buf is None else buf, name, t).cpu().numpy().copy()
                         for t in range(towers)]
        return out


def xavier_uniform(rng, fan_in, fan_out, shape):
    limit = math.sqrt(6.0 / (fan_in + fan_out))
    return rng.uniform(-limit, limit, size=shape).astype(np.float32)


def normalized_columns(std):
    def init(shape):
        out = np.random.randn(*shape).astype(np.float32)
        out *= std / np.sqrt(np.square(out).sum(axis=0, keepdims=True))
        return out
    return init


PAIR_GRADIENT_GEMMS = True
DIRECT_CONV_INPUT_GRAD = False
FUSE_CONV_PAIR = True
FUSE_CONV_FIRST = True
FUSE_CONV_INPUT_GRADS = True
FUSE_CONV_INPUT_GRADS_MIN_WORKGROUPS = 64
PER_RIDER_MAX_WORKGROUPS = 256
DENSE_DX_KW_MIN_TILES = 96
CONV1_CHUNKS = None
CONV_FORWARD_WAVE_GROUPS = 4


def _fused_operands_aligned(args):
    prev_tensor = False
    for a in args:
        if hasattr(a, "data_ptr"):
            if a.data_ptr() % 16:
                return False
            prev_tensor = True
        else:
            if prev_tensor and isinstance(a, int) and a % 4:
                return False
            prev_tensor = False
    return True


def _tiled_wave_groups(M, N, batch):
    if N <= 32:
        return 1
    below, least = ctypes.c_int(), ctypes.c_int()
    _rlx.lib().gemm_tuning_get(ctypes.byref(below), ctypes.byref(least), None)
    t64 = -(-M // 64) * -(-N // 64) * batch
    if t64 >= below.value:
        return 1
    if -(-M // 32) * -(-N // 64) * batch >= least.value:
        return 2
    if -(-M // 32) * -(-N // 32) * batch >= least.value:
        return 4
    return 1


def _kw2_tiling(M, N, batch):
    return _tiled_wave_groups(M, N, batch) == 2


MULTI_DW = False
SPLIT_CAP_BOUND = 128
CONV_DW_U8 = True
CONV_DW_F32 = True
CONV_DW_ONE_LAUNCH = True


class Workspace:
    def __init__(self, device, floats=1 << 24):
        self.splitk = torch.empty(floats, dtype=torch.float32, device=device)
        self.splitk_side = torch.empty(floats, dtype=torch.float32, device=device)
        self.small = torch.empty(1 << 18, dtype=torch.float32, device=device)


class Context:

    def __init__(self, device, ws=None):
        self.device = device
        self.lib = _rlx.lib()
        self.ws = ws or Workspace(device)
        self.cache = {}
        self.buffers = {}
        self.overlap = False
        self.deferred, self.arena, self._arena_off = None, None, 0

    @property
    def stream(self):
        return torch.cuda.current_stream().cuda_stream

    def join(self):
        pass

    ARENA_FLOATS = 1 << 25
    _arenas = {}
    private_arena = False

    def begin_deferring(self):
        if self.deferred is not None:
            return False
        if self.arena is None or (self.private_arena and self.arena is Context._arenas.get(str(self.device))):
            if self.private_arena:
                self.arena = torch.empty(self.ARENA_FLOATS, dtype=torch.float32, device=self.device)
            else:
                key = str(self.device)
                if key not in Context._arenas:
                    Context._arenas[key] = torch.empty(self.ARENA_FLOATS, dtype=torch.float32, device=self.device)
                self.arena = Context._arenas[key]
        self.deferred, self._arena_off = [], 0
        return True

    def deferred_workspace(self, M, N, batch):
        bound = (M * N + N) * batch * SPLIT_CAP_BOUND
        room = self.ARENA_FLOATS - self._arena_off
        if self.deferred is None or len(self.deferred) >= _rlx.MAX_SPLITK_JOBS or room < (M * N + N) * batch * 2:
            return None, self.ws.splitk
        return _rlx.SplitkJob(), self.arena[self._arena_off:self._arena_off + min(bound, room)]

    def commit_deferred(self, job, reserved=False):
        if job is not None and job.splits > 1:
            self.deferred.append(job)
            if not reserved:
                self._arena_off += (job.workspace_floats() + 3) // 4 * 4

    def reserve_deferred_workspace(self, M, N, batch):
        job, ws = self.deferred_workspace(M, N, batch)
        if job is not None:
            self._arena_off += (ws.numel() + 3) // 4 * 4
        return job, ws

    def flush_deferred(self):
        jobs, self.deferred = self.deferred, None
        tail, self.ppo_tail = self.ppo_tail, None
        per, self.per_tail = self.per_tail, None
        if jobs or tail is not None or per is not None:
            _rlx.splitk_reduce_jobs(jobs or [], self.stream, ppo_tail=tail, per_tail=per)

    ppo_tail = None
    per_tail = None

    def flush_ppo_tail(self):
        tail, self.ppo_tail = self.ppo_tail, None
        if tail is not None:
            self.lib.ppo_heads_tail(ctypes.byref(tail), self.stream)

    def buffer(self, name, shape, dtype=torch.float32, tag=""):
        key = (name, tuple(shape), dtype, tag)
        buf = self.buffers.get(key)
        if buf is None:
            buf = torch.empty(shape, dtype=dtype, device=self.device)
            self.buffers[key] = buf
        return buf


class Tensor:

    def __init__(self, data, rows, cols, towers, u8=False, div=1.0, grad_key=None, act=None):
        self.data, self.rows, self.cols, self.towers = data, rows, cols, towers
        self.u8, self.div = u8, div
        self.act = act
        self.grad_is_dz = False
        self.grad = None
        self.grad_key = grad_key
        self.bn_saved = None

    def tower_stride(self):
        return 0 if self.towers == 0 else self.rows * self.cols

    def ensure_grad(self):
        if self.grad is None:
            if self.grad_key is not None:
                ctx, name, tag = self.grad_key
                self.grad = ctx.buffer(name + ":grad", tuple(self.data.shape), tag=tag)
            else:
                self.grad = torch.empty(self.data.shape, dtype=torch.float32, device=self.data.device)
        return self.grad

    def tower(self, t):
        g = self.ensure_grad()
        v = Tensor(self.data[t:t + 1], self.rows, self.cols, 1, u8=self.u8, div=self.div, act=self.act)
        v.grad = g[t:t + 1]
        v.bn_saved = self.bn_saved
        return v

    def slice_towers(self, t0, n, with_grad=True):
        v = Tensor(self.data[t0:t0 + n], self.rows, self.cols, n, u8=self.u8, div=self.div, act=self.act)
        if with_grad:
            v.grad = self.ensure_grad()[t0:t0 + n]
        v.bn_saved = self.bn_saved
        return v

    def tower_view(self, t):
        return Tensor(self.data[t:t + 1], self.rows, self.cols, 1, u8=self.u8, div=self.div, act=self.act)


def input_tensor(data, rows, cols, u8=False, div=1.0):
    return Tensor(data, rows, cols, 0, u8=u8, div=div)


class Layer:
    def _range(self, t0, nt):
        nt = self.T - t0 if nt is None else nt
        assert 0 <= t0 and t0 + nt <= self.T
        return t0, nt


class Dense(Layer):

    def __init__(self, params, name, in_features, units, activation=None, towers=1, init=None):
        self.name, self.K, self.N, self.act, self.T = name, in_features, units, activation, towers
        self.init, self.params = init, params
        self.kname, self.bname = name + "/kernel", name + "/bias"
        params.add_group([(self.kname, (in_features, units)), (self.bname, (units,))], towers)

    def initialize(self, rng):
        for t in range(self.T):
            w = self.init((self.K, self.N)) if self.init is not None else \
                xavier_uniform(rng, self.K, self.N, (self.K, self.N))
            self.params.w(self.kname, t).copy_(torch.from_numpy(np.ascontiguousarray(w)))

    def forward(self, ctx, x, tag="", weights=None, t0=0, nt=None, pair=False, launch=True, row_heads=None):
        t0, T = self._range(t0, nt)
# ... 708 lines not shown
        if _rlx.GEMM_HOOK is not None:
            d2, d3 = _rlx.GemmDesc(), _rlx.GemmDesc()
            d2.M, d2.N, d2.K, d2.batch = M2, a.Co, a.K, T
            d3.M, d3.N, d3.K, d3.batch = M3, b.Co, b.K, T
            _rlx._record((d1, d2, d3), run)
        run()
        return [Tensor(y, B, l.OH * l.OW * l.Co, T, grad_key=(ctx, l.name, tag), act=l.act)
                for y, l in ((y1, f), (y2, a), (y3, b))]

    def _fused_conv_input_grads(self, ctx, acts, i, weights, t0, nt, kw, need_dx_below):
        b, a = self.layers[i], self.layers[i - 1]
        if not FUSE_CONV_INPUT_GRADS or not (isinstance(a, Conv2d) and isinstance(b, Conv2d)) or ctx.overlap or \
                not need_dx_below or a.T != b.T or a.direct_input_grad() or b.direct_input_grad():
            return False
        y3, x2, x1 = acts[i + 1], acts[i], acts[i - 1]
        t0_, T = b._range(t0, nt)
        B, p, lib = x2.rows, b.params, ctx.lib
        if x2.towers != T or x1.towers != T or x1.u8 or x2.act != x1.act or a.out_hwc != (b.H, b.W, b.C) or \
                2 * B * T < FUSE_CONV_INPUT_GRADS_MIN_WORKGROUPS or \
                not lib.conv32_input_grad_supported(a.H, a.W, a.C, a.KH, a.S, a.Co, b.KH, b.S, b.Co):
            return False
        M3, M2, M1 = B * b.OH * b.OW, B * a.OH * a.OW, B * a.H * a.W
        dz3 = y3.grad
        dz2, dz1 = x2.ensure_grad(), x1.ensure_grad()
        descs = []
        for l, M, dz in ((b, M3, dz3), (a, M2, dz2)):
            dcol = ctx.buffer(l.name + "/dcol", (T, M, l.K))
            d = _rlx.gemm(M, l.K, l.Co, dz, p.w(l.kname, t0_, weights), dcol, b_strides=(1, l.Co), batch=T,
                          a_batch_stride=M * l.Co, b_batch_stride=p.stride(l.kname), c_batch_stride=M * l.K,
                          workspace=ctx.ws.splitk, launch=False)
            q = (ctypes.c_int * 8)()
            lib.gemm_describe(ctypes.byref(d), q)
            fast, bm, bn, kwg, splits, kchunk, ring, thin = list(q)
            if not (fast and ring and not thin and kwg == 1 and splits == 1):
                return False
            descs.append(d)
        if b.act is not None and not y3.grad_is_dz:
            lib.act_backward(dz3, y3.data, dz3.numel(), _rlx.ACT[b.act], ctx.stream)
            y3.grad_is_dz = True
        args = (dz3, M3 * b.Co, p.w(b.kname, t0_, weights), p.stride(b.kname), x2.data, M2 * a.Co, dz2, M2 * a.Co,
                p.w(a.kname, t0_, weights), p.stride(a.kname), x1.data, M1 * a.C, dz1, M1 * a.C, B, T,
                _rlx.ACT[x2.act], ctx.stream)
        per, ctx.per_tail = ctx.per_tail, None
        if per is not None and 2 * B * T + 1 <= PER_RIDER_MAX_WORKGROUPS:
            pd = _rlx.per_update_desc(per)
            run = lambda: lib.conv32_input_grad_per_update(*args[:-1], ctypes.byref(pd), args[-1])
        else:
            ctx.per_tail = per
            run = lambda: lib.conv32_input_grad(*args)
        _rlx._record(tuple(descs), run)
        run()
        x2.grad_is_dz, x1.grad_is_dz = x2.act is not None, x1.act is not None
        if kw.get("need_dw", True):
            for l, x, y in ((b, x2, y3), (a, x1, x2)):
                l.backward(ctx, x, y, need_dx=False, weights=weights, t0=t0, nt=nt, **kw)
        return True

    def backward(self, ctx, acts, need_input_grad=False, weights=None, t0=0, nt=None, need_dw=True,
                 layers=None):
        lo, hi = layers if layers is not None else (0, len(self.layers))
        mine = need_dw and ctx.begin_deferring()
        try:
            later = [] if (MULTI_DW and need_dw and ctx.deferred is not None and not ctx.overlap and
                           sum(isinstance(self.layers[i], Conv2d) for i in range(lo, hi)) >= 2) else None
            collect = [] if (CONV_DW_ONE_LAUNCH and need_dw and later is None and ctx.deferred is not None and
                             not ctx.overlap) else None
            i = hi
            while i > lo:
                i -= 1
                kw = {"overlap": True} if need_dw else {"need_dw": False}
                if collect is not None and isinstance(self.layers[i], Conv2d):
                    kw["dw_collect"] = collect
                if i - 1 >= lo and later is None and \
                        self._fused_conv_input_grads(ctx, acts, i, weights, t0, nt, kw, i - 1 > 0 or need_input_grad):
                    i -= 1
                    continue
                if later is not None and isinstance(self.layers[i], Conv2d):
                    kw["dw_later"] = later
                self.layers[i].backward(ctx, acts[i], acts[i + 1], need_dx=(i > 0 or need_input_grad),
                                        weights=weights, t0=t0, nt=nt, **kw)
            while collect:
                group = sorted(collect[:3], key=lambda e: (not e[0].x_is_u8, -e[0].H))
                collect = collect[3:]
                _rlx.conv_dw_multi([it for it, _ in group], [j for _, j in group], ctx.stream)
                for _, j in group:
                    ctx.commit_deferred(j, reserved=True)
            while later:
                group, later = later[:3], later[3:]
                _rlx.gemm_multi([d for d, _ in group], [j for _, j in group])
                for _, j in group:
                    ctx.commit_deferred(j, reserved=True)
            ctx.join()
        finally:
            if mine:
                ctx.flush_deferred()


class AdamState:

    def __init__(self, params, lr, beta1=0.9, beta2=0.99, epsilon=1e-4):
        dev = params.weights.device
        self.params, self.lr, self.beta1, self.beta2, self.eps = params, lr, beta1, beta2, epsilon
        self.m = torch.empty_like(params.weights)
        self.v = torch.empty_like(params.weights)
        self.state = torch.empty(2, dtype=torch.float32, device=dev)
        self.ticket = torch.zeros(_rlx.ADAM_TICKET_WORDS, dtype=torch.int32, device=dev)
        self.one_launch = True
        _rlx.lib().adam_init(self.m, self.v, params.size, self.state, beta1, beta2, _rlx.current_stream())

    def step(self, grad_scale=1.0, lr=None, norm_out=None, workspace=None, acc=None, grads=None, mix_target=None,
             mix_rate=0.0):
        p = self.params
        lr = self.lr if lr is None else lr
        g = p.grads if grads is None else grads
        if self.one_launch:
            _rlx.lib().adam_tf1_step(p.weights, g, self.m, self.v, p.size, lr, self.beta1, self.beta2, self.eps,
                                     self.state, grad_scale, norm_out, workspace if norm_out is not None else None,
                                     workspace.numel() if norm_out is not None else 0,
                                     acc[0] if acc else None, acc[1] if acc else None, int(acc[2]) if acc else 0,
                                     mix_target, float(mix_rate), self.ticket, _rlx.current_stream())
            return
        if mix_target is not None:
            raise ValueError("the two-launch Adam path does not fuse the target update")
        if norm_out is not None:
            _rlx.lib().adam_tf1_norm(p.weights, g, self.m, self.v, p.size, lr, self.beta1,
                                     self.beta2, self.eps, self.state, grad_scale, norm_out, workspace,
                                     workspace.numel(), acc[0] if acc else None, acc[1] if acc else None,
                                     int(acc[2]) if acc else 0, _rlx.current_stream())
        else:
            _rlx.lib().adam_tf1(p.weights, g, self.m, self.v, p.size, lr, self.beta1, self.beta2,
                                self.eps, self.state, grad_scale, _rlx.current_stream())
```

### coach_amd/nn/networks.py

```python
import numpy as np
import torch

from .. import _rlx
from . import graph as G

IMAGE_EMBEDDER = {"Medium": [(32, 8, 4), (64, 4, 2), (64, 3, 1)], "Shallow": [(32, 3, 1)]}
VECTOR_EMBEDDER = {"Medium": [256], "Shallow": [128], "Empty": []}
FC_MIDDLEWARE = {"Medium": [512], "Shallow": [64], "Empty": []}


def build_torso(params, prefix, obs_shape, activation, towers, embedder="Medium", middleware="Medium", noisy=False):
    layers = []
    Dense = G.NoisyDense if noisy else G.Dense
    if len(obs_shape) == 3:
        hwc = tuple(obs_shape)
        convs = IMAGE_EMBEDDER[embedder] if isinstance(embedder, str) else embedder
        for i, (f, k, s) in enumerate(convs):
            c = G.Conv2d(params, "%s/embedder/conv%d" % (prefix, i), hwc, f, k, s, activation, towers)
            layers.append(c)
            hwc = c.out_hwc
        feat = hwc[0] * hwc[1] * hwc[2]
    else:
        feat = int(obs_shape[0])
        dense = VECTOR_EMBEDDER[embedder] if isinstance(embedder, str) else embedder
        for i, u in enumerate(dense):
            layers.append(Dense(params, "%s/embedder/dense%d" % (prefix, i), feat, u, activation, towers))
            feat = u
    mids = FC_MIDDLEWARE[middleware] if isinstance(middleware, str) else middleware
    for i, u in enumerate(mids):
        layers.append(Dense(params, "%s/middleware/dense%d" % (prefix, i), feat, u, activation, towers))
        feat = u
    return G.Sequential(layers), feat


class _NetBase:
    def _finish(self, device, seed, lr, beta1, beta2, eps, has_target=True):
        self.device = device
        self.params.finalize(device)
        rng = np.random.RandomState(seed)
        for m in self.modules:
            m.initialize(rng)
        self.ctx = G.Context(device)
        self.lib = self.ctx.lib
        self.adam = G.AdamState(self.params, lr, beta1, beta2, eps)
        if has_target:
            self.target = self.params.target_weights
            self.target.copy_(self.params.weights)
        else:
            self.target = None
        self.norm = torch.zeros(1, dtype=torch.float32, device=device)
        self.status = torch.zeros(1, dtype=torch.int32, device=device)

    def obs_tensor(self, obs, B):
        if self.image:
            return G.input_tensor(obs, B, int(np.prod(self.obs_shape)), u8=True, div=255.0)
        return G.input_tensor(obs, B, int(self.obs_shape[0]))

    def update_target(self, rate=1.0):
        self.lib.mix_weights(self.target, self.params.weights, self.params.size, float(rate), self.ctx.stream)

    def grad_norm(self):
        self.lib.global_norm(self.params.grads, self.params.size, self.norm, self.ctx.ws.small,
                             self.ctx.ws.small.numel(), self.ctx.stream)
        return self.norm

    def apply_gradients(self, grad_scale=1.0, with_norm=False, acc=None, mix_rate=None):
        kw = {}
        if mix_rate is not None and self.target is not None and self.adam.one_launch:
            kw = dict(mix_target=self.target, mix_rate=float(mix_rate))
        elif mix_rate is not None and self.target is not None:
            kw = {}
        if with_norm:
            self.adam.step(grad_scale, norm_out=self.norm, workspace=self.ctx.ws.small, acc=acc, **kw)
        else:
            self.adam.step(grad_scale, **kw)
        if mix_rate is not None and self.target is not None and not kw:
            self.update_target(mix_rate)
        for bn in getattr(self, "bn_layers", ()):
            bn.commit(self.ctx)

    def set_is_training(self, state):
        self.ctx.bn_training = bool(state)

    clip_gradients = None

    def clip_by_global_norm(self):
        if not self.clip_gradients:
            return False
        self.grad_norm()
        self.lib.clip_by_global_norm(self.params.grads, self.params.size, self.norm,
                                     float(self.clip_gradients), self.ctx.stream)
        return True

    def check_status(self):
        s = int(self.status.item())
        if s:
            self.status.zero_()
            raise ValueError("device kernel reported invalid input (status bits %d)" % s)


class ClippedPPONet(_NetBase):
    HEADS_LOSS_BACKWARD_ONE_LAUNCH = True
    HEADS_FORWARD_WITH_TORSO = True
    FC_HEADS_ONE_LAUNCH = False
    HEADS_ROW_LOCAL = True

    def __init__(self, device, obs_shape, n_actions, activation="tanh", embedder="Medium",
                 middleware="Medium", learning_rate=2.5e-4, adam_beta1=0.9, adam_beta2=0.99,
                 optimizer_epsilon=1e-4, clip_likelihood_ratio_using_epsilon=0.2, beta_entropy=0.01,
                 seed=0, continuous=False):
        self.obs_shape, self.image, self.A = tuple(obs_shape), len(obs_shape) == 3, n_actions
        self.clip_eps, self.beta = clip_likelihood_ratio_using_epsilon, beta_entropy
        self._clip_scale_dev, self._clip_scale_value = None, None
        self.continuous = continuous
        self.params = G.FlatParams()
        self.torso, feat = build_torso(self.params, "main", obs_shape, activation, 2, embedder, middleware)
        self.v_head = G.Dense(self.params, "main/v_head/dense", feat, 1, None, 1,
                              init=G.normalized_columns(1.0))
        if continuous:
            self.pi_head = G.Dense(self.params, "main/ppo_head/policy_mean", feat, n_actions, None, 1,
                                   init=G.normalized_columns(0.01))
            self.params.add_group([("main/ppo_head/policy_log_std", (n_actions,))])
        else:
            self.pi_head = G.Dense(self.params, "main/ppo_head/policy_fc", feat, n_actions, None, 1)
        self.modules = [self.torso, self.v_head, self.pi_head]
        self._finish(device, seed, learning_rate, adam_beta1, adam_beta2, optimizer_epsilon)
        self.scalars = torch.zeros(8, dtype=torch.float32, device=device)
        self.norm = self.scalars[5:6]

    def policy_probs(self, obs, B, use_target=False, tag="act", out=None, sample=None):
        w = self.target if use_target else None
        if self.HEADS_FORWARD_WITH_TORSO and self.pi_head.N <= G.SMALL_N and self.torso.layers[-1].N > G.SMALL_N:
            acts, (logits,) = self.torso.forward(self.ctx, self.obs_tensor(obs, B), tag=tag, weights=w, t0=1, nt=1,
                                                 row_heads=[(self.pi_head, 0)])
        else:
            acts = self.torso.forward(self.ctx, self.obs_tensor(obs, B), tag=tag, weights=w, t0=1, nt=1)
            logits = self.pi_head.forward(self.ctx, acts[-1], tag=tag, weights=w)
        if sample is not None:
            uniforms, actions = sample
            self.lib.softmax_categorical_sample(logits.data, self.A, uniforms, B, self.A, None, 0, actions, self.ctx.stream)
            return None
        probs = out if out is not None else self.ctx.buffer("probs", (B, self.A), tag=tag)
        self.lib.softmax(logits.data, self.A, B, self.A, probs, self.A, self.ctx.stream)
        return probs

    def act_and_record(self, obs, B, uniforms, actions, value_out, probs_out, tag="actrec"):
        ctx = self.ctx
        fused_heads = self.pi_head.N <= G.SMALL_N and B * self.pi_head.N <= 1024
        if fused_heads and self.HEADS_FORWARD_WITH_TORSO and self.torso.layers[-1].N > G.SMALL_N:
            acts, (v, logits) = self.torso.forward(ctx, self.obs_tensor(obs, B), tag=tag,
                                                   row_heads=[(self.v_head, 0, value_out), (self.pi_head, 1)])
        else:
            acts = self.torso.forward(ctx, self.obs_tensor(obs, B), tag=tag)
            mid = acts[-1]
            if fused_heads:
                v, logits = G.small_dense_forward_multi(ctx, [(self.v_head, mid.tower_view(0)), (self.pi_head, mid.tower_view(1))], tag=tag)
            else:
                v = self.v_head.forward(ctx, mid.tower_view(0), tag=tag)
                logits = self.pi_head.forward(ctx, mid.tower_view(1), tag=tag)
            value_out.copy_(v.data.view(-1))
        self.lib.softmax_categorical_sample(logits.data, self.A, uniforms, B, self.A, probs_out, self.A, actions, ctx.stream)

    def policy_mean_std(self, obs, B, use_target=False, tag="act", out_mean=None, out_std=None):
        w = self.target if use_target else None
        acts = self.torso.forward(self.ctx, self.obs_tensor(obs, B), tag=tag, weights=w, t0=1, nt=1)
        mean = self.pi_head.forward(self.ctx, acts[-1], tag=tag, weights=w).data.view(B, self.A)
        std = out_std if out_std is not None else self.ctx.buffer("policy_std", (B, self.A), tag=tag)
        ls = self.params.w("main/ppo_head/policy_log_std", 0, w)
        self.lib.exp_rows(ls, std, B, self.A, self.ctx.stream)
        if out_mean is not None:
            out_mean.copy_(mean)
            mean = out_mean
        return mean, std

    def values(self, obs, B, tag="val", out=None):
        if self.HEADS_FORWARD_WITH_TORSO and self.torso.layers[-1].N > G.SMALL_N:
            acts, (v,) = self.torso.forward(self.ctx, self.obs_tensor(obs, B), tag=tag, t0=0, nt=1,
                                            row_heads=[(self.v_head, 0)])
        else:
            acts = self.torso.forward(self.ctx, self.obs_tensor(obs, B), tag=tag, t0=0, nt=1)
            v = self.v_head.forward(self.ctx, acts[-1], tag=tag)
        if out is not None:
            out.copy_(v.data.view(-1))
            return out
        return v.data.view(-1)

    def late_gradient_offset(self):
        return self.params.entries[self.torso.layers[self._split_layer()].kname][0]

    def _split_layer(self):
        from .graph import Conv2d
        for i, l in enumerate(self.torso.layers):
            if not isinstance(l, Conv2d):
                return i
        return 0

    def set_clip_rescaler(self, value):
        if self._clip_scale_dev is None:
            self._clip_scale_dev = torch.ones(1, dtype=torch.float32, device=self.device)
        if self._clip_scale_value != float(value):
            self._clip_scale_dev.fill_(float(value))
            self._clip_scale_value = float(value)

    def forward_backward(self, obs, B, actions, advantages, value_targets, old_probs,
                         clip_rescaler=1.0, ratio_out=None, clipped_out=None, stop_after_dense=False):
        ctx = self.ctx
        clip_dev = self._clip_scale_dev if clip_rescaler is None else None
        if clip_rescaler is None:
            assert clip_dev is not None, "set_clip_rescaler first"
            clip_rescaler = 1.0
        fused_heads = self.pi_head.N <= G.SMALL_N and B * self.pi_head.N <= 1024
        heads_with_torso = fused_heads and self.HEADS_FORWARD_WITH_TORSO and self.torso.layers[-1].N > G.SMALL_N
        discrete_fused = heads_with_torso and not self.continuous and self.HEADS_LOSS_BACKWARD_ONE_LAUNCH
        if (self.FC_HEADS_ONE_LAUNCH or (self.HEADS_ROW_LOCAL and B <= 256)) and discrete_fused:
            acts = self.torso.forward(ctx, self.obs_tensor(obs, B), tag="train", skip_last=True)
            if self.HEADS_ROW_LOCAL and B <= 256 and not self.FC_HEADS_ONE_LAUNCH and len(acts) == len(self.torso.layers):
                res = G.ppo_fc_rows(ctx, self.torso.layers[-1], acts[-1], self.v_head, self.pi_head, value_targets, actions,
                                    advantages, old_probs, self.A, self.clip_eps * clip_rescaler, clip_dev, self.beta,
                                    self.scalars, ratio_out, clipped_out, self.status, tag="train",
                                    tail_now=stop_after_dense)
                if res is not None:
                    acts.append(res[0])
                    return self._backward_torso(acts, stop_after_dense)
            if self.FC_HEADS_ONE_LAUNCH and len(acts) == len(self.torso.layers) and \
                    G.ppo_fc_heads_supported(ctx, self.torso.layers[-1], acts[-1], self.v_head, self.pi_head):
                mid, v, logits = G.ppo_fc_heads(ctx, self.torso.layers[-1], acts[-1], self.v_head, self.pi_head, value_targets,
                                                actions, advantages, old_probs, self.A, self.clip_eps * clip_rescaler, clip_dev,
                                                self.beta, self.scalars, ratio_out, clipped_out, self.status, tag="train")
                acts.append(mid)
                return self._backward_torso(acts, stop_after_dense)
            last = self.torso.layers[-1]
            if heads_with_torso:
                y, (v, logits) = last.forward(ctx, acts[-1], tag="train", row_heads=[(self.v_head, 0), (self.pi_head, 1)])
            else:
                y = last.forward(ctx, acts[-1], tag="train")
            acts.append(y)
        elif heads_with_torso:
            acts, (v, logits) = self.torso.forward(ctx, self.obs_tensor(obs, B), tag="train",
                                                   row_heads=[(self.v_head, 0), (self.pi_head, 1)])
        else:
            acts = self.torso.forward(ctx, self.obs_tensor(obs, B), tag="train")
        mid = acts[-1]
        mid.ensure_grad()
        xv, xp = mid.tower(0), mid.tower(1)
        if heads_with_torso:
            pass
        elif fused_heads:
            v, logits = G.small_dense_forward_multi(ctx, [(self.v_head, xv), (self.pi_head, xp)], tag="train")
        else:
            v = self.v_head.forward(ctx, xv, tag="train")
            logits = self.pi_head.forward(ctx, xp, tag="train")
        one_launch = fused_heads and not self.continuous and B <= 256 and self.HEADS_LOSS_BACKWARD_ONE_LAUNCH
        if one_launch:
            G.ppo_heads_loss_backward(ctx, (self.v_head, xv, v), (self.pi_head, xp, logits), value_targets, actions,
                                      advantages, old_probs, self.A, self.clip_eps * clip_rescaler, clip_dev, self.beta,
                                      self.scalars, ratio_out, clipped_out, self.status)
        dv, dlogits = v.ensure_grad(), logits.ensure_grad()
        if one_launch:
            pass
        elif not self.continuous:
            self.lib.ppo_discrete_value_losses(logits.data, self.A, actions, advantages, old_probs, self.A, B,
                                               self.A, self.clip_eps * clip_rescaler, self.beta, 1.0, dlogits,
                                               self.A, self.scalars[0:4], ratio_out, clipped_out, self.status,
                                               v.data, value_targets, dv, self.scalars[4:5], clip_dev, ctx.stream)
        else:
            self.lib.regression_loss(v.data, 1, value_targets, 1, None, B, 1, 0, 1.0, 1.0, dv, 1,
                                     self.scalars[4:5], ctx.stream)
        if self.continuous:
            old_mean, old_std = old_probs
            self.lib.ppo_continuous_loss(logits.data, self.A, self.params.w("main/ppo_head/policy_log_std"),
                                         actions, advantages, old_mean, old_std, self.A, B, self.A,
                                         self.clip_eps * clip_rescaler, self.beta, 1.0, dlogits, self.A,
                                         self.params.g("main/ppo_head/policy_log_std"), self.scalars[0:4],
                                         ratio_out, clipped_out, clip_dev, ctx.stream)

        if one_launch:
            pass
        elif fused_heads:
            G.small_dense_backward_multi(ctx, [(self.v_head, xv, v), (self.pi_head, xp, logits)])
        else:
            self.v_head.backward(ctx, xv, v)
            self.pi_head.backward(ctx, xp, logits)
        mid.grad_is_dz = xv.grad_is_dz and xp.grad_is_dz
        self._backward_torso(acts, stop_after_dense)

    def _backward_torso(self, acts, stop_after_dense):
        ctx = self.ctx
        if stop_after_dense:
            k = self._split_layer()
            self.torso.backward(ctx, acts, layers=(k, len(self.torso.layers)))
            self._resume = (acts, k)
        else:
            self.torso.backward(ctx, acts)
        ctx.flush_ppo_tail()

    def backward_rest(self):
        acts, k = self._resume
        if k > 0:
            self.torso.backward(self.ctx, acts, layers=(0, k))

    def finish_update(self, grad_scale=1.0, signal_acc=None):
        self.apply_gradients(grad_scale, with_norm=True,
                             acc=(self.scalars, signal_acc, 6) if signal_acc is not None else None)

    def train_minibatch(self, obs, B, actions, advantages, value_targets, old_probs,
                        clip_rescaler=1.0, grad_scale=1.0, ratio_out=None, clipped_out=None):
        self.forward_backward(obs, B, actions, advantages, value_targets, old_probs, clip_rescaler,
                              ratio_out, clipped_out)
        self.finish_update(grad_scale)
        return self.scalars


class DQNNet(_NetBase):
    HEAD_FORWARD_WITH_TORSO = True
    HEAD_LOSS_BACKWARD_ONE_LAUNCH = True
    FUSED_MLP = True
    FUSED_ACT = True

    def __init__(self, device, obs_shape, n_actions, activation="relu", embedder="Medium",
                 middleware="Medium", learning_rate=2.5e-4, adam_beta1=0.9, adam_beta2=0.99,
                 optimizer_epsilon=1e-4, replace_mse_with_huber_loss=True, seed=0, dueling=False,
                 head_activation="relu", head_gradient_rescale=1.0, clip_gradients=None, noisy=False):
        self.obs_shape, self.image, self.A = tuple(obs_shape), len(obs_shape) == 3, n_actions
        self.huber = replace_mse_with_huber_loss
        self.dueling = dueling
        self.noisy = bool(noisy)
        self.head_gradient_rescale = float(head_gradient_rescale)
        self.clip_gradients = clip_gradients
        self.params = G.FlatParams()
        self.torso, feat = build_torso(self.params, "main", obs_shape, activation, 1, embedder, middleware,
                                       noisy=self.noisy)
        if dueling and self.noisy:
            hn = "main/dueling_q_values_head"
            self.v_fc = G.NoisyDense(self.params, hn + "/state_value/fc1", feat, 512, head_activation)
            self.a_fc = G.NoisyDense(self.params, hn + "/action_advantage/fc1", feat, 512, head_activation)
            self.v_out = G.NoisyDense(self.params, hn + "/state_value/fc2", 512, 1, None)
            self.a_out = G.NoisyDense(self.params, hn + "/action_advantage/fc2", 512, n_actions, None)
            self.modules = [self.torso, self.v_fc, self.a_fc, self.v_out, self.a_out]
        elif dueling:
            hn = "main/dueling_q_values_head"
            self.stream_fc = G.Dense(self.params, hn + "/fc1", feat, 512, head_activation, 2)
            self.v_out = G.Dense(self.params, hn + "/state_value/fc2", 512, 1, None, 1)
            self.a_out = G.Dense(self.params, hn + "/action_advantage/fc2", 512, n_actions, None, 1)
            self.modules = [self.torso, self.stream_fc, self.v_out, self.a_out]
        else:
            self.q_head = self._q_head_layer(feat, n_actions)
            self.modules = [self.torso, self.q_head]
        self._finish(device, seed, learning_rate, adam_beta1, adam_beta2, optimizer_epsilon)
        self.loss = torch.zeros(1, dtype=torch.float32, device=device)
        self._noisy_setup()
        self._fused = self._fused_mlp_setup()
        self._act = self._act_setup()

    def _q_head_layer(self, feat, units):
        return (G.NoisyDense if self.noisy else G.Dense)(self.params, "main/q_head/dense", feat, units, None, 1)

    def _noisy_setup(self):
        self.noisy_layers = [l for m in self.modules for l in (m.layers if isinstance(m, G.Sequential) else [m])
                             if isinstance(l, G.NoisyDense)]
        for i, l in enumerate(self.noisy_layers):
            l.index = i
        if len(self.noisy_layers) > _rlx.NOISY_MAX_LAYERS:
            raise ValueError("a noisy network may have at most %d dense layers (this one has %d)"
                             % (_rlx.NOISY_MAX_LAYERS, len(self.noisy_layers)))
        self.noise_seed, self.noise_rank = 0, 0
        self.noise_counters = torch.zeros(max(1, len(self.noisy_layers)) * _rlx.NOISY_PASSES, dtype=torch.int64,
                                          device=self.device) if self.noisy else None

    def sample_noise(self, tag, noise_pass):
        if not self.noisy:
            return
        key = ("noisy_layers", tag)
        arr = self.ctx.cache.get(key)
        if arr is None:
            arr = (_rlx.NoisyLayer * len(self.noisy_layers))()
            for q, l in zip(arr, self.noisy_layers):
                q.f, q.f64, q.K, q.N, q.layer = l.noise(self.ctx, tag).data_ptr(), None, l.K, l.N, l.index
            self.ctx.cache[key] = arr
        import ctypes
        self.lib.noisy_sample(ctypes.byref(arr), len(arr), self.noise_counters, _rlx.NOISY_PASS[noise_pass],
                              self.noise_seed, self.noise_rank, self.ctx.stream)

    def _fused_mlp_setup(self):
        if not self.FUSED_MLP or self.image or self.dueling:
            return None
        ls = self.torso.layers
        if len(ls) != 2 or any(not isinstance(l, G.Dense) or l.act != "relu" or l.T != 1 for l in ls):
            return None
        if self.head_gradient_rescale != 1.0 or self.clip_gradients:
            return None
        d0, h1, h2 = ls[0].K, ls[0].N, ls[1].N
# ... 116 lines not shown
        if self.dueling:
            self._dueling_backward(acts[-1], q, saved, B)
        else:
            self.q_head.backward(ctx, acts[-1], q)
        if self.head_gradient_rescale != 1.0:
            g = acts[-1].grad
            self.lib.axpby(g, self.head_gradient_rescale, g, 0.0, None, g.numel(), ctx.stream)
        self.torso.backward(ctx, acts)

    def accumulate_regression(self, obs, B, targets, importance_weights=None):
        ctx = self.ctx
        self.sample_noise("train", "online")
        acts = self.torso.forward(ctx, self.obs_tensor(obs, B), tag="train")
        saved = None
        if self.dueling:
            q, saved = self._dueling_forward(acts[-1], B, "train", train=True)
        else:
            q = self.q_head.forward(ctx, acts[-1], tag="train")
        self.lib.regression_loss(q.data, self.A, targets, self.A, importance_weights, B, self.A, int(self.huber),
                                 1.0, 1.0, q.ensure_grad(), self.A, self.loss, ctx.stream)
        self._backward_from_q(acts, q, saved, B)
        if not self.clip_by_global_norm():
            self.grad_norm()
        return self.loss

    def _online_and_target_forward(self, obs, next_obs, B, states_pair):
        ctx, saved = self.ctx, None
        if states_pair is not None and not self.dueling and not self.noisy:
            cols = int(np.prod(self.obs_shape))
            both = states_pair.view(2, B, cols)
            x = G.Tensor(both, B, cols, 2, u8=self.image, div=255.0 if self.image else 1.0)
            if self.HEAD_FORWARD_WITH_TORSO and self.A <= G.SMALL_N and self.q_head.T == 1 and \
                    self.torso.layers[-1].N > G.SMALL_N:
                acts2, (q2,) = self.torso.forward(ctx, x, tag="pair", pair=True, row_heads=[(self.q_head, "pair")])
            else:
                acts2 = self.torso.forward(ctx, x, tag="pair", pair=True)
                q2 = self.q_head.forward(ctx, acts2[-1], tag="pair", pair=True)
            q_next = q2.data[1].view(B, -1)
            acts = [x.tower_view(0)] + [a.tower(0) for a in acts2[1:]]
            q = q2.tower(0)
        else:
            q_next = self.q_values(next_obs, B, use_target=True, tag="next_t", noise_pass="target").data.view(B, -1)
            self.sample_noise("train", "online")
            acts = self.torso.forward(ctx, self.obs_tensor(obs, B), tag="train")
            if self.dueling:
                q, saved = self._dueling_forward(acts[-1], B, "train", train=True)
            else:
                q = self.q_head.forward(ctx, acts[-1], tag="train")
        return acts, q, saved, q_next

    def _apply_update(self, grad_scale, sync):
        clipped = self.clip_by_global_norm()
        if sync is not None:
            sync.all_reduce_sum(self.params.grads)
        self.apply_gradients(grad_scale, with_norm=not clipped)

    def learn_from_batch(self, obs, next_obs, B, actions, rewards, game_overs, discount,
                         importance_weights=None, td_errors=None, double_dqn=False, grad_scale=1.0,
                         sync=None, states_pair=None):
        ctx = self.ctx
        if self._fused is not None and sync is None and B <= 32 and obs.is_contiguous() and next_obs.is_contiguous():
            w = importance_weights
            if w is not None and w.dtype != torch.float64:
                w = w.double()
            return self._fused_learn(obs, next_obs, B, actions, rewards, game_overs, discount, w, td_errors,
                                     double_dqn, grad_scale)
        sel = self.q_values(next_obs, B, tag="next_o", noise_pass="online_next").data.view(B, self.A) \
            if double_dqn else None
        acts, q, saved, q_next = self._online_and_target_forward(obs, next_obs, B, states_pair)
        dq = q.ensure_grad()
        w = importance_weights
        if w is not None and w.dtype != torch.float64:
            w = w.double()
        feat = acts[-1]
        if self.HEAD_LOSS_BACKWARD_ONE_LAUNCH and not self.dueling and self.head_gradient_rescale == 1.0 and \
                self.q_head.T == 1 and self.A <= G.SMALL_N and B * self.A <= 1024 and B <= 256 and not feat.u8 and \
                feat.towers == 1 and not self.noisy:
            import ctypes
            prob = _rlx.SmallDenseProblem()
            G._small_backward_problem(prob, self.q_head, feat, q)
            self.lib.dqn_head_loss_backward(ctypes.byref(prob), q.data, self.A, q_next, sel, self.A, actions, rewards,
                                            game_overs, w, float(discount), B, self.A, int(self.huber), 1.0, td_errors,
                                            self.loss, self.status, ctx.stream)
            self.torso.backward(ctx, acts)
        else:
            self.lib.dqn_head_loss(q.data, self.A, q_next, sel, self.A, actions, rewards, game_overs, w,
                                   float(discount), B, self.A, int(self.huber), 1.0, dq, self.A, td_errors,
                                   None, self.A, self.loss, self.status, ctx.stream)
            self._backward_from_q(acts, q, saved, B)
        self._apply_update(grad_scale, sync)
        return self.loss


class DistributionalDQNNet(DQNNet):
    FUSED_MLP = False
    FUSED_ACT = False
    HEAD_FORWARD_WITH_TORSO = False

    def __init__(self, device, obs_shape, n_actions, atoms, **kw):
        kw.pop("replace_mse_with_huber_loss", None)
        kw.pop("dueling", None)
        super().__init__(device, obs_shape, n_actions * atoms, dueling=False, **kw)
        self.A, self.N, self.AN = n_actions, int(atoms), n_actions * int(atoms)
        self.loss_ws = torch.zeros(256, dtype=torch.float32, device=device)
        self.ticket = torch.zeros(1, dtype=torch.int32, device=device)

    def head_output(self, obs, B, use_target=False, tag="q", noise_pass="act"):
        return DQNNet.q_values(self, obs, B, use_target=use_target, tag=tag, noise_pass=noise_pass)

    def learn_from_batch(self, obs, next_obs, B, actions, rewards, game_overs, discount, grad_scale=1.0,
                         sync=None, states_pair=None, **head_outs):
        acts, q, _, q_next = self._online_and_target_forward(obs, next_obs, B, states_pair)
        dq = q.ensure_grad()
        self._head_loss(q.data, q_next, dq, actions, rewards, game_overs, float(discount), B, **head_outs)
        self._backward_from_q(acts, q, None, B)
        self._apply_update(grad_scale, sync)
        return self.loss


class QRDQNNet(DistributionalDQNNet):

    def __init__(self, device, obs_shape, n_actions, atoms, huber_loss_interval=1.0, **kw):
        super().__init__(device, obs_shape, n_actions, atoms, **kw)
        self.kappa = float(huber_loss_interval)

    quantiles = DistributionalDQNNet.head_output

    def _head_loss(self, q, q_next, dq, actions, rewards, game_overs, discount, B, targets_out=None, tau_out=None,
                   target_actions_out=None):
        AN = self.AN
        self.lib.qr_dqn_head_loss(q, AN, q_next, AN, actions, rewards, game_overs, discount, self.kappa, self.N, self.A,
                                  B, 1.0, dq, AN, self.loss_ws, self.ticket, self.loss, self.status, targets_out,
                                  tau_out, target_actions_out, self.ctx.stream)


class C51Net(DistributionalDQNNet):

    def __init__(self, device, obs_shape, n_actions, atoms, v_min=-10.0, v_max=10.0, **kw):
        super().__init__(device, obs_shape, n_actions, atoms, **kw)
        self.z_values = np.linspace(v_min, v_max, self.N)
        self.z = torch.from_numpy(self.z_values).to(device)

    distribution_logits = DistributionalDQNNet.head_output

    def _head_loss(self, q, q_next, dq, actions, rewards, game_overs, discount, B, per_errors=None, m_out=None,
                   target_actions_out=None, action_losses_out=None):
        AN = self.AN
        self.lib.c51_head_loss(q, AN, q_next, AN, self.z, actions, rewards, game_overs, discount, self.N, self.A, B, 1.0,
                               dq, AN, per_errors, self.loss_ws, self.ticket, self.loss, self.status, m_out,
                               target_actions_out, action_losses_out, self.ctx.stream)


class _HeadCopiesDense(G.Dense):

    def __init__(self, params, name, in_features, units, copies):
        super().__init__(params, name, in_features, units * copies, None, 1)
        self.units, self.copies = units, copies

    def initialize(self, rng):
        w = np.concatenate([G.xavier_uniform(rng, self.K, self.units, (self.K, self.units)) for _ in range(self.copies)],
                           axis=1)
        self.params.w(self.kname, 0).copy_(torch.from_numpy(np.ascontiguousarray(w)))


class BootstrappedDQNNet(DQNNet):
    FUSED_MLP = False
    FUSED_ACT = False
    HEAD_FORWARD_WITH_TORSO = False
    MAX_HEADS = 32

    def __init__(self, device, obs_shape, n_actions, heads, dueling=False, noisy=False, **kw):
        if dueling or noisy:
            raise ValueError("Bootstrapped DQN has plain Q heads: the reference has neither a dueling nor a noisy form")
# ... 178 lines not shown
```

### include/rlx.h

```cpp
#ifndef RLX_H
#define RLX_H

#include <stddef.h>
#include <stdint.h>

#ifdef __cplusplus
extern "C" {
#endif

typedef enum rlx_status {
    RLX_OK = 0,
    RLX_ERR_INVALID_ARG = -1,
    RLX_ERR_HIP = -2,
    RLX_ERR_UNSUPPORTED = -3
} rlx_status;

#define RLX_ABI_VERSION 11
int rlx_abi_version(void);
const char *rlx_last_error(void);
const char *rlx_build_arch(void);
int rlx_device_count(int *count_host);
int rlx_stream_sync(void *stream);
int rlx_event_create(void **event_host);
int rlx_event_destroy(void *event);
// ... 341 lines not shown
    const float *dy; long long dy_tower_stride;
    float *dw; long long dw_tower_stride;
    float *db; long long db_tower_stride;
    float *dx; long long dx_tower_stride;
    int towers, M, K, N, activation, lower_activation;
} rlx_small_dense_problem;
int rlx_dqn_head_loss_backward(const rlx_small_dense_problem *q_head, const float *q_online, long long ld_q,
                               const float *q_next_target, const float *q_next_selector, long long ld_next,
                               const int *actions, const float *rewards, const unsigned char *game_overs,
                               const double *importance_weights, double discount, int batch, int n_actions, int huber,
                               float grad_scale, double *td_errors, float *loss_scalar, int *status, void *stream);
int rlx_dense_small_forward_multi(const rlx_small_dense_problem *problems_host, int n_problems, void *stream);
int rlx_dense_small_backward_multi(const rlx_small_dense_problem *problems_host, int n_problems, void *stream);
int rlx_ppo_heads_loss_backward(const rlx_small_dense_problem *value_head, const rlx_small_dense_problem *policy_head,
                                const float *values, const float *value_targets, const float *logits,
                                const int *actions, const float *advantages, const float *old_probs, long long ld_old,
                                int batch, float clip_epsilon, const float *clip_scale, float beta_entropy,
                                float grad_scale, float *scalars, float *likelihood_ratio,
                                float *clipped_likelihood_ratio, int *status, void *stream);
typedef struct rlx_ppo_rows_desc {
    rlx_small_dense_problem value_head, policy_head;
    const float *value_targets;
    const int *actions;
    const float *advantages;
    const float *old_probs; long long ld_old;
    const float *clip_scale;
    float clip_epsilon, beta_entropy, grad_scale;
    int batch;
    float *row_terms;
    float *scalars;
    float *likelihood_ratio, *clipped_likelihood_ratio;
    int *status;
} rlx_ppo_rows_desc;
int rlx_ppo_fc_rows_supported(const rlx_gemm_desc *fc, int n_actions);
int rlx_ppo_fc_rows(const rlx_gemm_desc *fc, const rlx_ppo_rows_desc *rows, void *stream);
int rlx_ppo_heads_tail(const rlx_ppo_rows_desc *rows, void *stream);
int rlx_splitk_reduce_jobs_ppo_tail(const rlx_splitk_job *jobs_host, int n_jobs, const rlx_ppo_rows_desc *rows, void *stream);
int rlx_splitk_reduce_jobs_per_update(const rlx_splitk_job *jobs_host, int n_jobs, double *sum_tree, double *min_tree,
                                      double *max_tree, int capacity, const int *idx, const double *td_errors, int n,
                                      double alpha, double epsilon, double *max_priority, int *status, void *stream);

int rlx_regression_loss(const float *out, long long ld_out, const float *target,
                        long long ld_target, const float *importance_weights, int batch, int dim,
                        int kind, float loss_weight, float grad_scale, float *grad,
                        long long ld_grad, float *loss_scalar, void *stream);
int rlx_softmax(const float *logits, long long ld, int batch, int n, float *probs,
                long long ld_out, void *stream);
int rlx_ppo_discrete_loss(const float *logits, long long ld, const int *actions,
                          const float *advantages, const float *old_probs, long long ld_old,
                          int batch, int n_actions, float clip_epsilon, float beta_entropy,
                          float grad_scale, float *dlogits, long long ld_grad, float *scalars,
                          float *likelihood_ratio, float *clipped_likelihood_ratio, int *status,
                          const float *clip_scale, void *stream);

int rlx_ppo_discrete_value_losses(const float *logits, long long ld, const int *actions,
                                  const float *advantages, const float *old_probs, long long ld_old,
                                  int batch, int n_actions, float clip_epsilon, float beta_entropy,
                                  float grad_scale, float *dlogits, long long ld_grad, float *scalars,
                                  float *likelihood_ratio, float *clipped_likelihood_ratio, int *status,
                                  const float *values, const float *value_targets, float *dvalues,
                                  float *value_loss_scalar, const float *clip_scale, void *stream);

int rlx_ppo_continuous_loss(const float *mean, long long ld, const float *log_std, const float *actions,
                            const float *advantages, const float *old_mean, const float *old_std,
                            long long ld_old, int batch, int action_dim, float clip_epsilon,
                            float beta_entropy, float grad_scale, float *dmean, long long ld_grad,
                            float *dlog_std, float *scalars, float *likelihood_ratio,
                            float *clipped_likelihood_ratio, const float *clip_scale, void *stream);

int rlx_adam_init(float *m, float *v, long long n, float *state, float beta1, float beta2,
                  void *stream);
int rlx_adam_tf1(float *weights, const float *grads, float *m, float *v, long long n,
                 float learning_rate, float beta1, float beta2, float epsilon, float *state,
                 float grad_scale, void *stream);
int rlx_adam_tf1_norm(float *weights, const float *grads, float *m, float *v, long long n,
                      float learning_rate, float beta1, float beta2, float epsilon, float *state,
                      float grad_scale, float *norm_out, float *workspace, long long workspace_floats,
                      const float *acc_src, float *acc_dst, int n_acc, void *stream);
#define RLX_ADAM_TICKET_WORDS 1056
int rlx_adam_tf1_step(float *weights, const float *grads, float *m, float *v, long long n, float learning_rate,
                      float beta1, float beta2, float epsilon, float *state, float grad_scale, float *norm_out,
                      float *workspace, long long workspace_floats, const float *acc_src, float *acc_dst, int n_acc,
                      float *target, double mix_rate, unsigned int *ticket, void *stream);
int rlx_adam_norm_in_kernel(int on);
int rlx_mix_weights(float *target, const float *online, long long n, double rate,
                    void *stream);
int rlx_global_norm(const float *x, long long n, float *norm_out, float *workspace,
                    long long workspace_floats, void *stream);

int rlx_clip_by_global_norm(float *grads, long long n, const float *global_norm, float clip_norm,
                            void *stream);
int rlx_clip_by_value(float *grads, long long n, float clip_value, void *stream);

int rlx_copy_2d(const float *src, long long src_ld, float *dst, long long dst_ld, int rows, int cols,
                float scale, void *stream);
int rlx_exp_rows(const float *log_std, float *out, int batch, int action_dim,
                 void *stream);
int rlx_axpby(float *out, float a, const float *x, float b, const float *y, long long n,
              void *stream);
int rlx_min_pair(const float *q1, const float *q2, float *out_min, float *grad1, float *grad2,
                 float grad_scale, int n, void *stream);
int rlx_sac_min_targets(const float *q1, const float *q2, const float *sampled_logprob, float grad_scale, int n,
                        float *out_min, float *value_targets, float *grad1, float *grad2, void *stream);
int rlx_select_rows(const unsigned char *mask, const void *if_set, const void *if_clear, void *out,
                    int n, long long row_bytes, void *stream);
int rlx_sac_policy_head(const float *mu_logsig, long long ld, const double *standard_normals, int batch,
                        int action_dim, float *out_mean, float *out_log_std, float *out_raw_actions,
                        float *out_actions, float *out_logprob, void *stream);
int rlx_sac_policy_head_backward(const float *mu_logsig, long long ld, const double *standard_normals,
                                 int batch, int action_dim, float logprob_mean_weight,
                                 const float *action_weights, float action_weight_scale,
                                 float *d_mu_logsig, long long ld_grad, int accumulate, void *stream);

int rlx_categorical_sample(const float *probs, long long ld, const double *uniforms, int n_env,
                           int n_actions, int *actions, void *stream);
int rlx_softmax_categorical_sample(const float *logits, long long ld, const double *uniforms, int n_env,
                                   int n_actions, float *probs_out, long long ld_out, int *actions, void *stream);
int rlx_argmax_rows(const float *values, long long ld, int n_rows, int n_cols, int *out,
                    void *stream);
int rlx_egreedy(const float *q_values, long long ld, const double *explore_uniforms,
                const int *random_actions, const double *tie_break_uniforms, double epsilon,
                int n_env, int n_actions, int *actions, void *stream);
int rlx_gaussian_action(const float *mean, const float *std_per_dim, const float *std_per_sample,
                        const double *standard_normals, const float *action_low,
                        const float *action_high, int n_env, int action_dim, float *actions,
                        void *stream);

int rlx_qr_dqn_head_loss(const float *theta, long long ld_theta, const float *theta_next_target, long long ld_next,
                         const int *actions, const float *rewards, const unsigned char *game_overs, double discount,
                         float kappa, int n_atoms, int n_actions, int batch, float grad_scale, float *dtheta,
                         long long ld_dtheta, float *row_partials, unsigned int *ticket, float *loss_scalar,
                         int *status, float *targets_out, float *tau_out, int *target_actions_out, void *stream);
int rlx_quantile_egreedy(const float *quantiles, long long ld, int n_atoms, const double *explore_uniforms,
                         const int *random_actions, const double *tie_break_uniforms, double epsilon, int n_env,
                         int n_actions, double *q_out, int *actions, void *stream);

int rlx_c51_head_loss(const float *logits, long long ld_logits, const float *logits_next_target, long long ld_next,
                      const double *z, const int *actions, const float *rewards, const unsigned char *game_overs,
                      double discount, int n_atoms, int n_actions, int batch, float grad_scale, float *dlogits,
                      long long ld_dlogits, double *per_errors, float *row_partials, unsigned int *ticket,
                      float *loss_scalar, int *status, float *m_out, int *target_actions_out, float *action_losses_out,
                      void *stream);
int rlx_categorical_egreedy(const float *logits, long long ld, const double *z, int n_atoms,
                            const double *explore_uniforms, const int *random_actions,
                            const double *tie_break_uniforms, double epsilon, int n_env, int n_actions, double *q_out,
                            int *actions, void *stream);

int rlx_synth_env_reset(int kind, void *obs, int *episode, int *step, int n_env, int obs_elems,
                        unsigned int seed, unsigned int env_id0, void *stream);
int rlx_synth_env_step(int kind, void *next_obs, void *reset_obs, float *reward,
                       unsigned char *game_over, int *episode, int *step, int n_env, int obs_elems,
                       int episode_len, unsigned int seed, unsigned int env_id0, void *stream);

int rlx_synth_env_step_lengths(int kind, void *next_obs, void *reset_obs, float *reward,
                               unsigned char *game_over, int *episode, int *step, int n_env, int obs_elems,
                               const int *episode_len_per_env, unsigned int seed, unsigned int env_id0,
                               void *stream);

int rlx_normal_fill(double *out, const long long *events, int n_events, int stream0, int n_streams, int n,
                    unsigned int seed, unsigned int rank, double scale, void *stream);

#define RLX_NOISY_PASSES 4
#define RLX_NOISY_MAX_LAYERS 8
typedef struct rlx_noisy_layer {
    float *f;
    double *f64;
// ... 53 lines not shown
                       unsigned int env_id0, int next_episode, void *stream);
int rlx_cartpole_step(const int *action, double *state, int *episode, int *steps, float *next_obs, float *reset_obs,
                      double *next_state64, float *reward, unsigned char *game_over, int n_env,
                      int max_episode_steps, unsigned int seed, unsigned int env_id0, int *status, void *stream);
int rlx_libm_sincos(const double *x, double *sin_out, double *cos_out, int n, int *status, void *stream);


typedef struct rlx_mlp3 {
    long long off_w1, off_b1, off_w2, off_b2, off_w3, off_b3;
    long long tower_stride1, tower_stride2, tower_stride3;
    int d_in, h1, h2, d_out;
} rlx_mlp3;
typedef struct rlx_fused_net {
    float *weights, *target_weights, *adam_m, *adam_v, *adam_state, *grads, *norm_out;
    unsigned int *ticket;
    float learning_rate, beta1, beta2, epsilon, grad_scale, mix_rate;
} rlx_fused_net;
typedef struct rlx_td3_fused_desc {
    rlx_fused_net actor, critic;
    rlx_mlp3 actor_mlp, critic_mlp;
    const float *obs, *next_obs, *actions, *rewards;
    const unsigned char *game_overs;
    const double *noise;
    const float *action_low, *action_high;
    double noise_clip, discount, clip_low, clip_high;
    int use_non_zero_discount_for_terminal_states, has_clip;
    float actor_scale;
    int batch, obs_dim, act_dim;
    float *workspace; long long workspace_floats;
    float *td_targets, *q_min, *loss, *neg_action_grad;
} rlx_td3_fused_desc;
int rlx_td3_fused_supported(const rlx_td3_fused_desc *desc_host);
int rlx_fused_phase_stamps(int enable);
int rlx_td3_fused_workspace_floats(const rlx_td3_fused_desc *desc_host, long long *floats_host);
int rlx_td3_fused_critic_update(const rlx_td3_fused_desc *desc_host, int write_grads, void *stream);
int rlx_td3_fused_actor_update(const rlx_td3_fused_desc *desc_host, int write_grads, void *stream);


typedef struct rlx_sac_fused_desc {
    rlx_fused_net policy, q, v;
    rlx_mlp3 policy_mlp, v_mlp;
    long long q_off_obs_w, q_off_obs_b, q_off_act_w, q_off_act_b, q_off_fc_w, q_off_fc_b, q_off_out_w, q_off_out_b;
    long long q_stride_obs, q_stride_act, q_stride_fc, q_stride_out;
    const float *obs, *next_obs, *actions, *rewards;
    const unsigned char *game_overs;
    const double *normals;
    double discount;
    int resample_noise_per_pass, batch, obs_dim, act_dim, q_hidden, reserved;
    float *workspace; long long workspace_floats;
    float *value_targets, *log_target, *td_targets, *dq_da, *q_loss, *v_loss;
} rlx_sac_fused_desc;
int rlx_sac_fused_supported(const rlx_sac_fused_desc *desc_host);
int rlx_sac_fused_workspace_floats(const rlx_sac_fused_desc *desc_host, long long *floats_host);
int rlx_sac_fused_update(const rlx_sac_fused_desc *desc_host, int write_grads, void *stream);

int rlx_conv_dw_u8_supported(int B, int H, int W, int C, int KH, int KW, int S, int filters, int towers);
int rlx_conv_dw_u8_workspace_floats(int B, int H, int W, int C, int KH, int KW, int S, int filters, int towers,
                                    long long *floats_host);
int rlx_conv_dw_u8(const unsigned char *frames, float a_div, const float *dz, long long dz_tower_stride, int B, int H, int W,
                   int C, int KH, int KW, int S, int filters, int towers, float *dw, long long dw_tower_stride, float *db,
                   long long db_tower_stride, float *workspace, long long workspace_floats, rlx_splitk_job *job_host,
                   void *stream);
int rlx_conv_dw_u8_stamps(long long *device_words5);

int rlx_conv_dw_f32_supported(int B, int H, int W, int C, int KH, int KW, int S, int filters, int towers);
int rlx_conv_dw_f32_workspace_floats(int B, int H, int W, int C, int KH, int KW, int S, int filters, int towers,
                                     long long *floats_host);
int rlx_conv_dw_f32(const float *x, long long x_tower_stride, const float *dz, long long dz_tower_stride, int B, int H, int W,
                    int C, int KH, int KW, int S, int filters, int towers, float *dw, long long dw_tower_stride, float *db,
                    long long db_tower_stride, float *workspace, long long workspace_floats, rlx_splitk_job *job_host,
                    void *stream);
int rlx_conv_dw_f32_stamps(long long *device_words4);

typedef struct rlx_conv_dw_item {
    const void *x; long long x_tower_stride;
    int x_is_u8; float a_div;
    const float *dz; long long dz_tower_stride;
    int B, H, W, C, KH, KW, S, filters, towers;
    float *dw; long long dw_tower_stride;
    float *db; long long db_tower_stride;
    float *workspace; long long workspace_floats;
} rlx_conv_dw_item;
int rlx_conv_dw_multi(const rlx_conv_dw_item *items_host, rlx_splitk_job *jobs_host, int n_items, void *stream);
int rlx_conv_dw_passes(int passes);
int rlx_conv_dw_pairs_per_workgroup(int pairs);

typedef struct rlx_ppo_fc_heads_desc {
    const float *x; long long x_tower_stride;
    const float *weights; long long weight_tower_stride;
    const float *bias; long long bias_tower_stride;
    const float *value_w, *value_b, *policy_w, *policy_b;
    const float *value_targets, *advantages, *old_probs; long long ld_old;
    const int *actions;
    const float *clip_scale;
    float clip_epsilon, beta_entropy, grad_scale;
    int batch, in_features, units, n_actions, activation;
    float *h, *dz, *values, *logits, *dvalues, *dlogits;
    float *d_value_w, *d_value_b, *d_policy_w, *d_policy_b;
    float *scalars, *likelihood_ratio, *clipped_likelihood_ratio;
    int *status;
    float *workspace; long long workspace_floats;
    unsigned int *tickets;
} rlx_ppo_fc_heads_desc;
int rlx_ppo_fc_heads_supported(int batch, int in_features, int units, int n_actions);
int rlx_ppo_fc_heads_workspace(int units, long long *floats_host, long long *ticket_words_host);
int rlx_ppo_fc_heads(const rlx_ppo_fc_heads_desc *desc_host, void *stream);
int rlx_ppo_fc_heads_stamps(int enable);

#ifdef __cplusplus
}
#endif
#endif
```

Baseline: 38620 env-steps/s.

## Fold split-K gradient reductions into Adam step and fuse PPO heads tail into conv dW

Split-K conv weight-gradient reductions are now held instead of launched, and the fused Adam+norm kernel sums the partials directly while reading gradients. It also writes the reduced gradients back to the grads buffer. Separately, the PPO value/policy heads backward tail is launched as extra workgroups inside the multi-item conv dW kernel instead of as its own kernel. Both aim to cut kernel launches and one full pass over gradient memory per minibatch. The cost is more complex holding/flush logic, a larger LDS request for the fused kernel, and fallbacks when regions fail alignment or overlap checks.

```diff
diff --git a/coach_amd/_rlx.py b/coach_amd/_rlx.py
--- a/coach_amd/_rlx.py
+++ b/coach_amd/_rlx.py
@@ -351,14 +351,17 @@
     return it
 
 
-def conv_dw_multi(items, jobs, stream=None):
+def conv_dw_multi(items, jobs, stream=None, ppo_tail=None):
     s = current_stream() if stream is None else stream
     n = len(items)
     arr = (ConvDwItem * n)(*items)
     jarr = (SplitkJob * n)()
 
     def run():
-        lib().conv_dw_multi(arr, jarr, n, s)
+        if ppo_tail is not None:
+            lib().conv_dw_multi_ppo_tail(arr, jarr, n, ctypes.byref(ppo_tail), s)
+        else:
+            lib().conv_dw_multi(arr, jarr, n, s)
     if GEMM_HOOK is not None:
         descs = []
         for it in items:
diff --git a/coach_amd/agents/clipped_ppo_agent.py b/coach_amd/agents/clipped_ppo_agent.py
--- a/coach_amd/agents/clipped_ppo_agent.py
+++ b/coach_amd/agents/clipped_ppo_agent.py
@@ -524,19 +524,21 @@
         return e
 
     def _minibatch_fb(self, m, clip_rescaler, stop_after_dense=False, i=0, epoch=None):
+        hold = self.dist is None and not stop_after_dense
         if epoch is not None:
             B = self.ap.network_wrappers["main"].batch_size
             sl = slice(i * B, i * B + m)
             old = (epoch["old"][sl], epoch["old_std"][sl]) if self.continuous else epoch["old"][sl]
             self.networks["main"].forward_backward(epoch["obs"][sl], m, epoch["action"][sl], epoch["adv"][sl],
                                                    epoch["vtarget"][sl], old, clip_rescaler, self.mb_ratio,
-                                                   self.mb_clipped, stop_after_dense=stop_after_dense)
+                                                   self.mb_clipped, stop_after_dense=stop_after_dense,
+                                                   hold_reductions=hold)
             return
         obs = self._gather_minibatch(m, i)
         old = (self.mb_old, self.mb_old_std) if self.continuous else self.mb_old
         self.networks["main"].forward_backward(obs, m, self.mb_action, self.mb_adv, self.mb_vtarget,
                                                old, clip_rescaler, self.mb_ratio, self.mb_clipped,
-                                               stop_after_dense=stop_after_dense)
+                                               stop_after_dense=stop_after_dense, hold_reductions=hold)
 
     def _minibatch_finish(self, scale):
         net = self.networks["main"]
diff --git a/coach_amd/csrc/conv_dw_multi.hip b/coach_amd/csrc/conv_dw_multi.hip
--- a/coach_amd/csrc/conv_dw_multi.hip
+++ b/coach_amd/csrc/conv_dw_multi.hip
@@ -1,4 +1,5 @@
 #include "conv_dw_body.hpp"
+#include "ppo_tail_body.hpp"
 
 namespace {
 
@@ -12,9 +13,7 @@
 };
 
 template <int PASSES>
-__global__ void __launch_bounds__(kThreads) conv_dw_multi_kernel(const MultiArgs m) {
-    extern __shared__ __attribute__((aligned(16))) float smem[];
-    int bid = blockIdx.x;
+__device__ __forceinline__ void conv_dw_multi_body(const MultiArgs &m, int bid, float *smem) {
     if (bid < m.nb_u8) {
         if (m.u8_half) conv_dw_u8_body_half(m.u8, bid, smem);
         else if constexpr (PASSES > 1) conv_dw_u8_body_passes<PASSES>(m.u8, bid, smem);
@@ -37,6 +36,24 @@
         bid -= m.nb_f[i];
     }
 }
+template <int PASSES>
+__global__ void __launch_bounds__(kThreads) conv_dw_multi_kernel(const MultiArgs m) {
+    extern __shared__ __attribute__((aligned(16))) float smem[];
+    conv_dw_multi_body<PASSES>(m, blockIdx.x, smem);
+}
+static_assert(kThreads == 256, "ppo_heads_tail_body: 256 threads");
+constexpr size_t kTailLds = sizeof(float) * (rlx_ppo_tail::kTailSmemFloats + rlx_ppo_tail::kTailRedFloats);
+template <int PASSES, int NN>
+__global__ void __launch_bounds__(kThreads) conv_dw_multi_tail_kernel(const MultiArgs m, const rlx_ppo_tail::PpoTailDev tail, int kb) {
+    extern __shared__ __attribute__((aligned(16))) float smem[];
+    const int bid = blockIdx.x;
+    if (bid < 2 * kb) {
+        float (*red)[256] = reinterpret_cast<float (*)[256]>(smem + rlx_ppo_tail::kTailSmemFloats);
+        rlx_ppo_tail::ppo_heads_tail_body<NN>(tail, bid < kb ? bid : bid - kb, bid >= kb, smem, red);
+        return;
+    }
+    conv_dw_multi_body<PASSES>(m, bid - 2 * kb, smem);
+}
 
 int g_passes = 2;
 int g_pairs_per_wg = 0;
@@ -48,9 +65,8 @@
 
 }
 
-extern "C" {
-
-int rlx_conv_dw_multi(const rlx_conv_dw_item *items, rlx_splitk_job *jobs, int n_items, void *stream) {
+static int conv_dw_multi_impl(const rlx_conv_dw_item *items, rlx_splitk_job *jobs, int n_items, const rlx_ppo_rows_desc *rows,
+                              void *stream) {
     RLX_REQUIRE(items && jobs && n_items >= 1 && n_items <= 3, "rlx_conv_dw_multi: 1 .. 3 items");
     int n_u8 = 0, n_f = 0;
     bool one = n_items >= 2;
@@ -83,7 +99,7 @@
                                   it.db_tower_stride, it.workspace, it.workspace_floats, &jobs[i], stream);
             if (rc != RLX_OK) return rc;
         }
-        return RLX_OK;
+        return rows ? rlx_ppo_heads_tail(rows, stream) : RLX_OK;
     }
     MultiArgs m;
     m.nb_u8 = m.nb_f[0] = m.nb_f[1] = 0;
@@ -147,6 +163,10 @@
         configured = true;
     }
     const unsigned grid = m.nb_u8 + m.nb_f[0] + m.nb_f[1];
+    if (rows && g_passes != 2) {
+        const int rc = conv_dw_multi_impl(items, jobs, n_items, nullptr, stream);
+        return rc != RLX_OK ? rc : rlx_ppo_heads_tail(rows, stream);
+    }
     if (g_passes > 1) {
         size_t lds2 = iu ? (m.u8_half ? lds_u8_half() : (g_passes == 4 ? lds_u8_passes<4>() : lds_u8_passes<2>())) : 0;
         for (int k = 0; k < 2; ++k) {
@@ -154,13 +174,44 @@
             const size_t l = m.kind[k] == 2 ? lds_f32_two_pass<32, 20, 9, 5>() : lds_f32_two_pass<64, 9, 7, 4>();
             lds2 = l > lds2 ? l : lds2;
         }
-        if (g_passes == 4) RLX_LAUNCH((conv_dw_multi_kernel<4>), grid, kThreads, lds2, rlx::as_stream(stream), m);
+        if (rows) {
+            static bool tail_configured = false;
+            if (!tail_configured) {
+                RLX_HIP(hipFuncSetAttribute(reinterpret_cast<const void *>(conv_dw_multi_tail_kernel<2, 4>),
+                                            hipFuncAttributeMaxDynamicSharedMemorySize, 160 * 1024));
+                RLX_HIP(hipFuncSetAttribute(reinterpret_cast<const void *>(conv_dw_multi_tail_kernel<2, 8>),
+                                            hipFuncAttributeMaxDynamicSharedMemorySize, 160 * 1024));
+                RLX_HIP(hipFuncSetAttribute(reinterpret_cast<const void *>(conv_dw_multi_tail_kernel<2, 16>),
+                                            hipFuncAttributeMaxDynamicSharedMemorySize, 160 * 1024));
+                tail_configured = true;
+            }
+            const rlx_ppo_tail::PpoTailDev t = rlx_ppo_tail::ppo_tail_dev(*rows);
+            const int kb = (rows->value_head.K + rlx_small::kKL - 1) / rlx_small::kKL;
+            lds2 = kTailLds > lds2 ? kTailLds : lds2;
+            hipStream_t s = rlx::as_stream(stream);
+            if (t.nn == 4) RLX_LAUNCH((conv_dw_multi_tail_kernel<2, 4>), grid + 2 * kb, kThreads, lds2, s, m, t, kb);
+            else if (t.nn == 8) RLX_LAUNCH((conv_dw_multi_tail_kernel<2, 8>), grid + 2 * kb, kThreads, lds2, s, m, t, kb);
+            else RLX_LAUNCH((conv_dw_multi_tail_kernel<2, 16>), grid + 2 * kb, kThreads, lds2, s, m, t, kb);
+        } else if (g_passes == 4) RLX_LAUNCH((conv_dw_multi_kernel<4>), grid, kThreads, lds2, rlx::as_stream(stream), m);
         else RLX_LAUNCH((conv_dw_multi_kernel<2>), grid, kThreads, lds2, rlx::as_stream(stream), m);
     } else {
         RLX_LAUNCH((conv_dw_multi_kernel<1>), grid, kThreads, lds, rlx::as_stream(stream), m);
     }
     RLX_LAUNCH_CHECK();
     return RLX_OK;
+}
+
+extern "C" {
+
+int rlx_conv_dw_multi(const rlx_conv_dw_item *items, rlx_splitk_job *jobs, int n_items, void *stream) {
+    return conv_dw_multi_impl(items, jobs, n_items, nullptr, stream);
+}
+
+int rlx_conv_dw_multi_ppo_tail(const rlx_conv_dw_item *items, rlx_splitk_job *jobs, int n_items, const rlx_ppo_rows_desc *rows,
+                               void *stream) {
+    const int rc0 = rlx_ppo_tail::ppo_rows_check(rows, "rlx_conv_dw_multi_ppo_tail");
+    if (rc0 != RLX_OK) return rc0;
+    return conv_dw_multi_impl(items, jobs, n_items, rows, stream);
 }
 
 int rlx_conv_dw_pairs_per_workgroup(int pairs) {
diff --git a/coach_amd/csrc/gemm.hip b/coach_amd/csrc/gemm.hip
--- a/coach_amd/csrc/gemm.hip
+++ b/coach_amd/csrc/gemm.hip
@@ -1,6 +1,7 @@
 #include "rlx_common.hpp"
 #include "dense_small_body.hpp"
 #include "losses_body.hpp"
+#include "ppo_tail_body.hpp"
 #include "splitk_reduce_body.hpp"
 #include <cstdlib>
 
@@ -1711,39 +1712,9 @@
     }
 }
 
-struct PpoTailDev {
-    rlx_small::SmallDenseBwd value, policy;
-    const float *row_terms;
-    float *scalars;
-    int batch, red_threads, nn;
-    float beta;
-};
-template <int NN>
-__device__ __forceinline__ void ppo_heads_tail_body(const PpoTailDev &a, int kblock, bool is_policy, float *smem,
-                                                    float (*red)[256]) {
-    using namespace rlx_losses;
-    const rlx_small::SmallDenseBwd &p = is_policy ? a.policy : a.value;
-    if (kblock * rlx_small::kKL >= p.K) return;
-    if (kblock == 0) {
-        const int b = threadIdx.x, B = a.batch;
-        if (is_policy) {
-            float l_sur = 0.f, l_ent = 0.f, l_kl = 0.f;
-            if (b < B) {
-                l_sur = a.row_terms[(size_t)b * 4 + 1];
-                l_ent = a.row_terms[(size_t)b * 4 + 2];
-                l_kl = a.row_terms[(size_t)b * 4 + 3];
-            }
-            block_sum3_first(l_sur, l_ent, l_kl, red, a.red_threads);
-            if (threadIdx.x == 0) ppo_discrete_scalars(l_sur, l_ent, l_kl, a.beta, B, a.scalars);
-        } else {
-            const float local = b < B ? a.row_terms[(size_t)b * 4] : 0.f;
-            const float s = block_sum_first(local, red[0], a.red_threads);
-            if (threadIdx.x == 0) a.scalars[4] = s / (float)B;
-        }
-    }
-    rlx_small::dense_small_bwd_body<NN, rlx_small::kKL, rlx_small::kRG, false>(p, kblock, 0, smem);
-}
-constexpr int kTailSmemFloats = 256 * rlx_small::kMaxN + rlx_small::kRG * rlx_small::kKL * rlx_small::kMaxN;
+using rlx_ppo_tail::PpoTailDev;
+using rlx_ppo_tail::ppo_heads_tail_body;
+using rlx_ppo_tail::kTailSmemFloats;
 
 template <int NN>
 __global__ void __launch_bounds__(256) ppo_heads_tail_kernel(const PpoTailDev a) {
@@ -2443,35 +2414,8 @@
 }
 
 namespace {
-int ppo_rows_check(const rlx_ppo_rows_desc *q, const char *who) {
-    RLX_REQUIRE(q && q->value_targets && q->actions && q->advantages && q->old_probs && q->row_terms && q->scalars &&
-                q->status, "%s: null pointer", who);
-    const rlx_small_dense_problem *h[2] = {&q->value_head, &q->policy_head};
-    for (int i = 0; i < 2; ++i) {
-        RLX_REQUIRE(h[i]->x && h[i]->w && h[i]->y && h[i]->dy && h[i]->dw && h[i]->dx, "%s: null pointer in head %d", who, i);
-        RLX_REQUIRE(h[i]->towers == 1 && h[i]->M == q->batch && h[i]->K > 0 && h[i]->activation == 0,
-                    "%s: head %d must be one linear tower over the %d rows of the batch", who, i, q->batch);
-        RLX_REQUIRE(h[i]->lower_activation >= 0 && h[i]->lower_activation <= 2, "%s: unknown activation", who);
-    }
-    RLX_REQUIRE(q->value_head.N == 1 && q->policy_head.N >= 2 && q->policy_head.N <= rlx_small::kMaxN &&
-                q->value_head.K == q->policy_head.K && q->value_head.lower_activation == q->policy_head.lower_activation,
-                "%s: value head N = 1, policy head 2 <= N <= %d, both on the same dense layer", who, rlx_small::kMaxN);
-    RLX_REQUIRE(q->batch >= 1 && q->batch <= 256, "%s: 1 <= batch <= 256 (one row per thread in the scalar sums)", who);
-    return RLX_OK;
-}
-PpoTailDev ppo_tail_dev(const rlx_ppo_rows_desc &q) {
-    PpoTailDev t{};
-    const rlx_small_dense_problem *h[2] = {&q.value_head, &q.policy_head};
-    rlx_small::SmallDenseBwd *d[2] = {&t.value, &t.policy};
-    for (int i = 0; i < 2; ++i)
-        *d[i] = rlx_small::SmallDenseBwd{h[i]->x, 0, h[i]->w, 0, h[i]->dy, 0, nullptr, 0, h[i]->dw, 0, h[i]->db, 0, nullptr, 0,
-                                         h[i]->M, h[i]->K, h[i]->N, 0, 0};
-    t.row_terms = q.row_terms; t.scalars = q.scalars; t.batch = q.batch; t.beta = q.beta_entropy;
-    t.red_threads = 64;
-    while (t.red_threads < q.batch) t.red_threads <<= 1;
-    t.nn = q.policy_head.N <= 4 ? 4 : (q.policy_head.N <= 8 ? 8 : 16);
-    return t;
-}
+using rlx_ppo_tail::ppo_rows_check;
+using rlx_ppo_tail::ppo_tail_dev;
 }
 
 int rlx_ppo_fc_rows_supported(const rlx_gemm_desc *fc, int n_actions) {
diff --git a/coach_amd/csrc/optim.hip b/coach_amd/csrc/optim.hip
--- a/coach_amd/csrc/optim.hip
+++ b/coach_amd/csrc/optim.hip
@@ -1,4 +1,6 @@
 #include "rlx_common.hpp"
+#include "splitk_reduce_body.hpp"
+#include <type_traits>
 
 namespace {
 
@@ -159,12 +161,15 @@
 }
 
 constexpr int kNormIt = 4;
-template <bool MIX>
+struct NoSources {};
+template <bool MIX, bool JOBS>
 __global__ void __launch_bounds__(kBlock)
-adam_step_norm_kernel(float *__restrict__ w, const float *__restrict__ g, float *__restrict__ m, float *__restrict__ v,
+adam_step_norm_kernel(float *__restrict__ w, std::conditional_t<JOBS, float, const float> *__restrict__ g,
+                      float *__restrict__ m, float *__restrict__ v,
                       long long n, float lr, float beta1, float beta2, float eps, float *state, float grad_scale,
                       float *sumsq_part, float *__restrict__ target, float rate, float one_minus_rate,
-                      unsigned int *ticket, float *norm_out, const float *acc_src, float *acc_dst, int n_acc) {
+                      unsigned int *ticket, float *norm_out, const float *acc_src, float *acc_dst, int n_acc,
+                      const std::conditional_t<JOBS, rlx_reduce::GradSources, NoSources> src) {
     __shared__ float red[kBlock];
     __shared__ int last_s;
     const float b1p = state[0], b2p = state[1];
@@ -174,11 +179,23 @@
     const long long n4 = n >> 2;
     const long long i0 = (long long)blockIdx.x * blockDim.x + threadIdx.x;
     float4 gw[kNormIt], mw[kNormIt], vw[kNormIt], ww[kNormIt], tw[kNormIt];
+    [[maybe_unused]] bool summed[kNormIt];
+    if constexpr (JOBS) {
+#pragma unroll
+        for (int it = 0; it < kNormIt; ++it) {
+            const long long i = i0 + it * stride;
+            summed[it] = i < n4 && rlx_reduce::grad_from_partials(src, i << 2, gw[it]);
+        }
+    }
 #pragma unroll
     for (int it = 0; it < kNormIt; ++it) {
         const long long i = i0 + it * stride;
         if (i < n4) {
-            gw[it] = reinterpret_cast<const float4 *>(g)[i];
+            if constexpr (JOBS) {
+                if (!summed[it]) gw[it] = reinterpret_cast<const float4 *>(g)[i];
+            } else {
+                gw[it] = reinterpret_cast<const float4 *>(g)[i];
+            }
             mw[it] = reinterpret_cast<float4 *>(m)[i];
             vw[it] = reinterpret_cast<float4 *>(v)[i];
             ww[it] = reinterpret_cast<float4 *>(w)[i];
@@ -224,6 +241,11 @@
             reinterpret_cast<float4 *>(w)[i] = ww[it];
             if (MIX) reinterpret_cast<float4 *>(target)[i] = tw[it];
         }
+    }
+    if constexpr (JOBS) {
+#pragma unroll
+        for (int it = 0; it < kNormIt; ++it)
+            if (summed[it]) reinterpret_cast<float4 *>(g)[i0 + it * stride] = gw[it];
     }
     if (has_tail) {
         const float gr = gt * grad_scale;
@@ -344,6 +366,55 @@
 }
 
 int g_norm_in_kernel = 2;
+
+bool grad_sources(const rlx_splitk_job *jobs, int n_jobs, const float *grads, long long n, rlx_reduce::GradSources *out) {
+    using rlx_reduce::GradRegion;
+    rlx_reduce::GradSources &t = *out;
+    t.n = 0; t.lo = n; t.hi = 0;
+    if (!jobs || n_jobs < 0 || n_jobs > RLX_MAX_SPLITK_JOBS || !grads) return false;
+    auto add = [&](const float *dst, long long len, const float *part, long long split_stride, int splits, int ld, int pn,
+                   int col0) {
+        if (t.n >= rlx_reduce::kMaxGradRegions || dst < grads || len <= 0) return false;
+        const long long begin = dst - grads, end = begin + len;
+        if (end > n || ((begin | end | split_stride | (long long)ld | (long long)pn | (long long)col0) & 3) != 0 ||
+            (((uintptr_t)part) & 15) != 0)
+            return false;
+        for (int i = 0; i < t.n; ++i)
+            if (begin < t.r[i].end && t.r[i].begin < end) return false;
+        t.r[t.n++] = GradRegion{begin, end, part, split_stride, splits, ld, pn, col0};
+        t.lo = begin < t.lo ? begin : t.lo;
+        t.hi = end > t.hi ? end : t.hi;
+        return true;
+    };
+    for (int i = 0; i < n_jobs; ++i) {
+        const rlx_splitk_job &j = jobs[i];
+        if (j.splits <= 1) continue;
+        if (!j.partials || !j.C || j.M <= 0 || j.N <= 0 || j.batch <= 0 || (long long)j.M * j.N >= (1LL << 31)) return false;
+        const long long mn = (long long)j.M * j.N;
+        const bool folded = j.n_fold > 0;
+        if (folded ? (j.batch != 1 || j.ldc != j.n_fold || j.N % j.n_fold != 0) : (j.ldc != j.N)) return false;
+        const int towers = folded ? j.N / j.n_fold : j.batch, cols = folded ? j.n_fold : j.N;
+        if (j.colsum_out && !j.colsum_partials) return false;
+        for (int tw = 0; tw < towers; ++tw) {
+            const float *part = folded ? j.partials : j.partials + (size_t)tw * j.splits * mn;
+            if (!add(j.C + (size_t)tw * j.c_batch_stride, (long long)j.M * cols, part, mn, j.splits, cols, j.N,
+                     folded ? tw * j.n_fold : 0))
+                return false;
+            if (j.colsum_out) {
+                const float *cp = folded ? j.colsum_partials : j.colsum_partials + (size_t)tw * j.splits * j.N;
+                if (!add(j.colsum_out + (size_t)tw * j.colsum_batch_stride, cols, cp, j.N, j.splits, cols, j.N,
+                         folded ? tw * j.n_fold : 0))
+                    return false;
+            }
+        }
+    }
+    return true;
+}
+inline int norm_blocks(long long n, long long workspace_floats) {
+    int blocks = rlx::grid_for(n / 4 + 1, kBlock, 1024);
+    if (blocks > workspace_floats) blocks = (int)workspace_floats;
+    return blocks;
+}
 }
 
 extern "C" {
@@ -425,11 +496,11 @@
                                                                   target, rate, omr, ticket, nullptr, nullptr, nullptr, 0)
     if (norm_out && g_norm_in_kernel == 2 && (n >> 2) <= (long long)blocks * kBlock * kNormIt) {
         if (target)
-            RLX_LAUNCH((adam_step_norm_kernel<true>), blocks, kBlock, 0, s, weights, grads, m, v, n, learning_rate, beta1, beta2,
-                       epsilon, state, grad_scale, workspace, target, rate, omr, ticket, norm_out, acc_src, acc_dst, n_acc);
+            RLX_LAUNCH((adam_step_norm_kernel<true, false>), blocks, kBlock, 0, s, weights, grads, m, v, n, learning_rate, beta1, beta2,
+                       epsilon, state, grad_scale, workspace, target, rate, omr, ticket, norm_out, acc_src, acc_dst, n_acc, NoSources{});
         else
-            RLX_LAUNCH((adam_step_norm_kernel<false>), blocks, kBlock, 0, s, weights, grads, m, v, n, learning_rate, beta1, beta2,
-                       epsilon, state, grad_scale, workspace, target, rate, omr, ticket, norm_out, acc_src, acc_dst, n_acc);
+            RLX_LAUNCH((adam_step_norm_kernel<false, false>), blocks, kBlock, 0, s, weights, grads, m, v, n, learning_rate, beta1, beta2,
+                       epsilon, state, grad_scale, workspace, target, rate, omr, ticket, norm_out, acc_src, acc_dst, n_acc, NoSources{});
         RLX_LAUNCH_CHECK();
         return RLX_OK;
     }
@@ -459,6 +530,42 @@
     return RLX_OK;
 }
 
+int rlx_adam_tf1_step_jobs_supported(const rlx_splitk_job *jobs_host, int n_jobs, const float *grads, long long n,
+                                     int with_norm, long long workspace_floats) {
+    if (!with_norm || n <= 0 || g_norm_in_kernel != 2) return 0;
+    const int blocks = norm_blocks(n, workspace_floats);
+    if (blocks < 1 || (n >> 2) > (long long)blocks * kBlock * kNormIt) return 0;
+    rlx_reduce::GradSources t;
+    return grad_sources(jobs_host, n_jobs, grads, n, &t) ? 1 : 0;
+}
+
+int rlx_adam_tf1_step_jobs(const rlx_splitk_job *jobs_host, int n_jobs, float *weights, float *grads, float *m, float *v,
+                           long long n, float learning_rate, float beta1, float beta2, float epsilon, float *state,
+                           float grad_scale, float *norm_out, float *workspace, long long workspace_floats,
+                           const float *acc_src, float *acc_dst, int n_acc, float *target, double mix_rate,
+                           unsigned int *ticket, void *stream) {
+    RLX_REQUIRE(weights && grads && m && v && state && ticket && norm_out && workspace, "rlx_adam_tf1_step_jobs: null pointer");
+    RLX_REQUIRE(n_acc == 0 || (acc_src && acc_dst && n_acc > 0 && n_acc <= 64),
+                "rlx_adam_tf1_step_jobs: bad signal accumulation arguments");
+    RLX_REQUIRE((((uintptr_t)weights | (uintptr_t)grads | (uintptr_t)m | (uintptr_t)v | (uintptr_t)target) & 15) == 0,
+                "rlx_adam_tf1_step_jobs: buffers must be 16-byte aligned");
+    rlx_reduce::GradSources t;
+    RLX_REQUIRE(rlx_adam_tf1_step_jobs_supported(jobs_host, n_jobs, grads, n, 1, workspace_floats) &&
+                    grad_sources(jobs_host, n_jobs, grads, n, &t),
+                "rlx_adam_tf1_step_jobs: not a case rlx_adam_tf1_step_jobs_supported accepts");
+    const int blocks = norm_blocks(n, workspace_floats);
+    hipStream_t s = rlx::as_stream(stream);
+    const float rate = (float)mix_rate, omr = (float)(1.0 - mix_rate);
+    if (target)
+        RLX_LAUNCH((adam_step_norm_kernel<true, true>), blocks, kBlock, 0, s, weights, grads, m, v, n, learning_rate, beta1, beta2,
+                   epsilon, state, grad_scale, workspace, target, rate, omr, ticket, norm_out, acc_src, acc_dst, n_acc, t);
+    else
+        RLX_LAUNCH((adam_step_norm_kernel<false, true>), blocks, kBlock, 0, s, weights, grads, m, v, n, learning_rate, beta1, beta2,
+                   epsilon, state, grad_scale, workspace, target, rate, omr, ticket, norm_out, acc_src, acc_dst, n_acc, t);
+    RLX_LAUNCH_CHECK();
+    return RLX_OK;
+}
+
 int rlx_mix_weights(float *target, const float *online, long long n, double rate, void *stream) {
     RLX_REQUIRE(target && online && n > 0, "rlx_mix_weights: bad arguments");
     RLX_REQUIRE((((uintptr_t)target | (uintptr_t)online) & 15) == 0,
diff --git a/coach_amd/csrc/ppo_tail_body.hpp b/coach_amd/csrc/ppo_tail_body.hpp
--- /dev/null
+++ b/coach_amd/csrc/ppo_tail_body.hpp
@@ -0,0 +1,73 @@
+#pragma once
+#include "rlx_common.hpp"
+#include "dense_small_body.hpp"
+#include "losses_body.hpp"
+
+namespace rlx_ppo_tail {
+
+struct PpoTailDev {
+    rlx_small::SmallDenseBwd value, policy;
+    const float *row_terms;
+    float *scalars;
+    int batch, red_threads, nn;
+    float beta;
+};
+template <int NN>
+__device__ __forceinline__ void ppo_heads_tail_body(const PpoTailDev &a, int kblock, bool is_policy, float *smem,
+                                                    float (*red)[256]) {
+    using namespace rlx_losses;
+    const rlx_small::SmallDenseBwd &p = is_policy ? a.policy : a.value;
+    if (kblock * rlx_small::kKL >= p.K) return;
+    if (kblock == 0) {
+        const int b = threadIdx.x, B = a.batch;
+        if (is_policy) {
+            float l_sur = 0.f, l_ent = 0.f, l_kl = 0.f;
+            if (b < B) {
+                l_sur = a.row_terms[(size_t)b * 4 + 1];
+                l_ent = a.row_terms[(size_t)b * 4 + 2];
+                l_kl = a.row_terms[(size_t)b * 4 + 3];
+            }
+            block_sum3_first(l_sur, l_ent, l_kl, red, a.red_threads);
+            if (threadIdx.x == 0) ppo_discrete_scalars(l_sur, l_ent, l_kl, a.beta, B, a.scalars);
+        } else {
+            const float local = b < B ? a.row_terms[(size_t)b * 4] : 0.f;
+            const float s = block_sum_first(local, red[0], a.red_threads);
+            if (threadIdx.x == 0) a.scalars[4] = s / (float)B;
+        }
+    }
+    rlx_small::dense_small_bwd_body<NN, rlx_small::kKL, rlx_small::kRG, false>(p, kblock, 0, smem);
+}
+constexpr int kTailSmemFloats = 256 * rlx_small::kMaxN + rlx_small::kRG * rlx_small::kKL * rlx_small::kMaxN;
+constexpr int kTailRedFloats = 3 * 256;
+
+inline int ppo_rows_check(const rlx_ppo_rows_desc *q, const char *who) {
+    RLX_REQUIRE(q && q->value_targets && q->actions && q->advantages && q->old_probs && q->row_terms && q->scalars &&
+                q->status, "%s: null pointer", who);
+    const rlx_small_dense_problem *h[2] = {&q->value_head, &q->policy_head};
+    for (int i = 0; i < 2; ++i) {
+        RLX_REQUIRE(h[i]->x && h[i]->w && h[i]->y && h[i]->dy && h[i]->dw && h[i]->dx, "%s: null pointer in head %d", who, i);
+        RLX_REQUIRE(h[i]->towers == 1 && h[i]->M == q->batch && h[i]->K > 0 && h[i]->activation == 0,
+                    "%s: head %d must be one linear tower over the %d rows of the batch", who, i, q->batch);
+        RLX_REQUIRE(h[i]->lower_activation >= 0 && h[i]->lower_activation <= 2, "%s: unknown activation", who);
+    }
+    RLX_REQUIRE(q->value_head.N == 1 && q->policy_head.N >= 2 && q->policy_head.N <= rlx_small::kMaxN &&
+                q->value_head.K == q->policy_head.K && q->value_head.lower_activation == q->policy_head.lower_activation,
+                "%s: value head N = 1, policy head 2 <= N <= %d, both on the same dense layer", who, rlx_small::kMaxN);
+    RLX_REQUIRE(q->batch >= 1 && q->batch <= 256, "%s: 1 <= batch <= 256 (one row per thread in the scalar sums)", who);
+    return RLX_OK;
+}
+inline PpoTailDev ppo_tail_dev(const rlx_ppo_rows_desc &q) {
+    PpoTailDev t{};
+    const rlx_small_dense_problem *h[2] = {&q.value_head, &q.policy_head};
+    rlx_small::SmallDenseBwd *d[2] = {&t.value, &t.policy};
+    for (int i = 0; i < 2; ++i)
+        *d[i] = rlx_small::SmallDenseBwd{h[i]->x, 0, h[i]->w, 0, h[i]->dy, 0, nullptr, 0, h[i]->dw, 0, h[i]->db, 0, nullptr, 0,
+                                         h[i]->M, h[i]->K, h[i]->N, 0, 0};
+    t.row_terms = q.row_terms; t.scalars = q.scalars; t.batch = q.batch; t.beta = q.beta_entropy;
+    t.red_threads = 64;
+    while (t.red_threads < q.batch) t.red_threads <<= 1;
+    t.nn = q.policy_head.N <= 4 ? 4 : (q.policy_head.N <= 8 ? 8 : 16);
+    return t;
+}
+
+}
diff --git a/coach_amd/csrc/splitk_reduce_body.hpp b/coach_amd/csrc/splitk_reduce_body.hpp
--- a/coach_amd/csrc/splitk_reduce_body.hpp
+++ b/coach_amd/csrc/splitk_reduce_body.hpp
@@ -76,4 +76,85 @@
     }
 }
 
+constexpr int kSplitGroups = 16;
+template <int ROUNDS>
+__device__ __forceinline__ float4 splitk_sum16_rounds(const float *base, size_t stride, int splits) {
+    constexpr int SG = kSplitGroups, U = 8 / ROUNDS;
+    float4 v = make_float4(0.f, 0.f, 0.f, 0.f);
+#pragma nounroll
+    for (int q0 = 0; q0 < SG; q0 += U) {
+        float4 p[U][ROUNDS];
+#pragma unroll
+        for (int g = 0; g < U; ++g)
+#pragma unroll
+            for (int j = 0; j < ROUNDS; ++j) {
+                const int k = q0 + g + j * SG;
+                const int kk = (j < ROUNDS - 1 || k < splits) ? k : splits - 1;
+                p[g][j] = *reinterpret_cast<const float4 *>(base + (size_t)kk * stride);
+            }
+#pragma unroll
+        for (int g = 0; g < U; ++g) {
+            float4 s = make_float4(0.f, 0.f, 0.f, 0.f);
+#pragma unroll
+            for (int j = 0; j < ROUNDS; ++j) {
+                const bool in = j < ROUNDS - 1 || q0 + g + j * SG < splits;
+                s.x = in ? s.x + p[g][j].x : s.x; s.y = in ? s.y + p[g][j].y : s.y;
+                s.z = in ? s.z + p[g][j].z : s.z; s.w = in ? s.w + p[g][j].w : s.w;
+            }
+            const bool first = q0 + g == 0;
+            v.x = first ? s.x : v.x + s.x; v.y = first ? s.y : v.y + s.y;
+            v.z = first ? s.z : v.z + s.z; v.w = first ? s.w : v.w + s.w;
+        }
+    }
+    return v;
 }
+__device__ __forceinline__ float4 splitk_sum16_any(const float *base, size_t stride, int splits) {
+    constexpr int SG = kSplitGroups;
+    float4 v = make_float4(0.f, 0.f, 0.f, 0.f);
+#pragma nounroll
+    for (int q = 0; q < SG; ++q) {
+        float4 s = make_float4(0.f, 0.f, 0.f, 0.f);
+        for (int k = q; k < splits; k += SG) {
+            const float4 a = *reinterpret_cast<const float4 *>(base + (size_t)k * stride);
+            s.x += a.x; s.y += a.y; s.z += a.z; s.w += a.w;
+        }
+        v.x = q == 0 ? s.x : v.x + s.x; v.y = q == 0 ? s.y : v.y + s.y;
+        v.z = q == 0 ? s.z : v.z + s.z; v.w = q == 0 ? s.w : v.w + s.w;
+    }
+    return v;
+}
+__device__ __forceinline__ float4 splitk_sum16_f4(const float *base, size_t stride, int splits) {
+    constexpr int SG = kSplitGroups;
+    if (splits <= SG) return splitk_sum16_rounds<1>(base, stride, splits);
+    if (splits <= 2 * SG) return splitk_sum16_rounds<2>(base, stride, splits);
+    if (splits > 3 * SG && splits <= 4 * SG) return splitk_sum16_rounds<4>(base, stride, splits);
+    return splitk_sum16_any(base, stride, splits);
+}
+
+struct GradRegion {
+    long long begin, end;
+    const float *part;
+    long long split_stride;
+    int splits, ld, pn, col0;
+};
+constexpr int kMaxGradRegions = 4 * RLX_MAX_SPLITK_JOBS;
+struct GradSources {
+    GradRegion r[kMaxGradRegions];
+    long long lo, hi;
+    int n;
+};
+__device__ __forceinline__ bool grad_from_partials(const GradSources &src, long long e, float4 &g) {
+    if (e < src.lo || e >= src.hi) return false;
+    for (int i = 0; i < src.n; ++i) {
+        const GradRegion &r = src.r[i];
+        if (e >= r.begin && e < r.end) {
+            const long long o = e - r.begin;
+            const long long row = o / r.ld;
+            g = splitk_sum16_f4(r.part + row * r.pn + r.col0 + (o - row * r.ld), (size_t)r.split_stride, r.splits);
+            return true;
+        }
+    }
+    return false;
+}
+
+}
diff --git a/coach_amd/nn/graph.py b/coach_amd/nn/graph.py
--- a/coach_amd/nn/graph.py
+++ b/coach_amd/nn/graph.py
@@ -134,6 +134,7 @@
 CONV_DW_U8 = True
 CONV_DW_F32 = True
 CONV_DW_ONE_LAUNCH = True
+REDUCE_IN_ADAM = True
 
 
 class Workspace:
@@ -176,6 +177,7 @@
                 if key not in Context._arenas:
                     Context._arenas[key] = torch.empty(self.ARENA_FLOATS, dtype=torch.float32, device=self.device)
                 self.arena = Context._arenas[key]
+        Context.flush_holder(self.arena)
         self.deferred, self._arena_off = [], 0
         return True
 
@@ -207,6 +209,38 @@
 
     ppo_tail = None
     per_tail = None
+
+    hold_reductions = False
+    held = None
+    _holders = {}
+
+    def holding(self):
+        return REDUCE_IN_ADAM and self.hold_reductions and self.per_tail is None
+
+    def end_deferring(self, failed=False):
+        if failed or not self.holding() or not self.deferred:
+            self.flush_deferred()
+            return
+        self.flush_ppo_tail()
+        self.held, self.deferred = self.deferred, None
+        Context._holders[self.arena.data_ptr()] = self
+
+    def take_held(self):
+        jobs, self.held = self.held, None
+        if jobs is not None:
+            Context._holders.pop(self.arena.data_ptr(), None)
+        return jobs
+
+    def flush_held(self):
+        jobs = self.take_held()
+        if jobs:
+            _rlx.splitk_reduce_jobs(jobs, self.stream)
+
+    @staticmethod
+    def flush_holder(arena):
+        h = Context._holders.get(arena.data_ptr()) if arena is not None else None
+        if h is not None:
+            h.flush_held()
 
     def flush_ppo_tail(self):
         tail, self.ppo_tail = self.ppo_tail, None
@@ -1081,7 +1115,10 @@
             while collect:
                 group = sorted(collect[:3], key=lambda e: (not e[0].x_is_u8, -e[0].H))
                 collect = collect[3:]
-                _rlx.conv_dw_multi([it for it, _ in group], [j for _, j in group], ctx.stream)
+                tail = ctx.ppo_tail if not collect and ctx.holding() else None
+                if tail is not None:
+                    ctx.ppo_tail = None
+                _rlx.conv_dw_multi([it for it, _ in group], [j for _, j in group], ctx.stream, ppo_tail=tail)
                 for _, j in group:
                     ctx.commit_deferred(j, reserved=True)
             while later:
@@ -1090,9 +1127,12 @@
                 for _, j in group:
                     ctx.commit_deferred(j, reserved=True)
             ctx.join()
-        finally:
+        except BaseException:
             if mine:
-                ctx.flush_deferred()
+                ctx.end_deferring(failed=True)
+            raise
+        if mine:
+            ctx.end_deferring()
 
 
 class AdamState:
@@ -1107,11 +1147,26 @@
         self.one_launch = True
         _rlx.lib().adam_init(self.m, self.v, params.size, self.state, beta1, beta2, _rlx.current_stream())
 
+    def step_jobs_supported(self, jobs, norm_out, workspace, grads=None):
+        if not jobs or not self.one_launch or norm_out is None or workspace is None or len(jobs) > _rlx.MAX_SPLITK_JOBS:
+            return False
+        p = self.params
+        arr = (_rlx.SplitkJob * len(jobs))(*jobs)
+        return bool(_rlx.lib().adam_tf1_step_jobs_supported(arr, len(jobs), _rlx._ptr(p.grads if grads is None else grads),
+                                                            p.size, 1, workspace.numel()))
+
     def step(self, grad_scale=1.0, lr=None, norm_out=None, workspace=None, acc=None, grads=None, mix_target=None,
-             mix_rate=0.0):
+             mix_rate=0.0, jobs=None):
         p = self.params
         lr = self.lr if lr is None else lr
         g = p.grads if grads is None else grads
+        if jobs:
+            arr = (_rlx.SplitkJob * len(jobs))(*jobs)
+            _rlx.lib().adam_tf1_step_jobs(arr, len(jobs), p.weights, g, self.m, self.v, p.size, lr, self.beta1, self.beta2,
+                                          self.eps, self.state, grad_scale, norm_out, workspace, workspace.numel(),
+                                          acc[0] if acc else None, acc[1] if acc else None, int(acc[2]) if acc else 0,
+                                          mix_target, float(mix_rate), self.ticket, _rlx.current_stream())
+            return
         if self.one_launch:
             _rlx.lib().adam_tf1_step(p.weights, g, self.m, self.v, p.size, lr, self.beta1, self.beta2, self.eps,
                                      self.state, grad_scale, norm_out, workspace if norm_out is not None else None,
diff --git a/coach_amd/nn/networks.py b/coach_amd/nn/networks.py
--- a/coach_amd/nn/networks.py
+++ b/coach_amd/nn/networks.py
@@ -60,18 +60,23 @@
         self.lib.mix_weights(self.target, self.params.weights, self.params.size, float(rate), self.ctx.stream)
 
     def grad_norm(self):
+        self.ctx.flush_held()
         self.lib.global_norm(self.params.grads, self.params.size, self.norm, self.ctx.ws.small,
                              self.ctx.ws.small.numel(), self.ctx.stream)
         return self.norm
 
     def apply_gradients(self, grad_scale=1.0, with_norm=False, acc=None, mix_rate=None):
+        held = self.ctx.take_held()
+        if held and not (with_norm and self.adam.step_jobs_supported(held, self.norm, self.ctx.ws.small)):
+            _rlx.splitk_reduce_jobs(held, self.ctx.stream)
+            held = None
         kw = {}
         if mix_rate is not None and self.target is not None and self.adam.one_launch:
             kw = dict(mix_target=self.target, mix_rate=float(mix_rate))
         elif mix_rate is not None and self.target is not None:
             kw = {}
         if with_norm:
-            self.adam.step(grad_scale, norm_out=self.norm, workspace=self.ctx.ws.small, acc=acc, **kw)
+            self.adam.step(grad_scale, norm_out=self.norm, workspace=self.ctx.ws.small, acc=acc, jobs=held or None, **kw)
         else:
             self.adam.step(grad_scale, **kw)
         if mix_rate is not None and self.target is not None and not kw:
@@ -203,7 +208,20 @@
             self._clip_scale_value = float(value)
 
     def forward_backward(self, obs, B, actions, advantages, value_targets, old_probs,
-                         clip_rescaler=1.0, ratio_out=None, clipped_out=None, stop_after_dense=False):
+                         clip_rescaler=1.0, ratio_out=None, clipped_out=None, stop_after_dense=False,
+                         hold_reductions=False):
+        self.ctx.hold_reductions = bool(hold_reductions) and not stop_after_dense
+        try:
+            return self._forward_backward(obs, B, actions, advantages, value_targets, old_probs, clip_rescaler, ratio_out,
+                                          clipped_out, stop_after_dense)
+        except BaseException:
+            self.ctx.flush_held()
+            raise
+        finally:
+            self.ctx.hold_reductions = False
+
+    def _forward_backward(self, obs, B, actions, advantages, value_targets, old_probs, clip_rescaler, ratio_out, clipped_out,
+                          stop_after_dense):
         ctx = self.ctx
         clip_dev = self._clip_scale_dev if clip_rescaler is None else None
         if clip_rescaler is None:
@@ -300,13 +318,17 @@
             self.torso.backward(self.ctx, acts, layers=(0, k))
 
     def finish_update(self, grad_scale=1.0, signal_acc=None):
-        self.apply_gradients(grad_scale, with_norm=True,
-                             acc=(self.scalars, signal_acc, 6) if signal_acc is not None else None)
+        try:
+            self.apply_gradients(grad_scale, with_norm=True,
+                                 acc=(self.scalars, signal_acc, 6) if signal_acc is not None else None)
+        except BaseException:
+            self.ctx.take_held()
+            raise
 
     def train_minibatch(self, obs, B, actions, advantages, value_targets, old_probs,
                         clip_rescaler=1.0, grad_scale=1.0, ratio_out=None, clipped_out=None):
         self.forward_backward(obs, B, actions, advantages, value_targets, old_probs, clip_rescaler,
-                              ratio_out, clipped_out)
+                              ratio_out, clipped_out, hold_reductions=True)
         self.finish_update(grad_scale)
         return self.scalars
 
@@ -589,13 +611,25 @@
             self.lib.dqn_head_loss_backward(ctypes.byref(prob), q.data, self.A, q_next, sel, self.A, actions, rewards,
                                             game_overs, w, float(discount), B, self.A, int(self.huber), 1.0, td_errors,
                                             self.loss, self.status, ctx.stream)
-            self.torso.backward(ctx, acts)
+            hold = True
         else:
             self.lib.dqn_head_loss(q.data, self.A, q_next, sel, self.A, actions, rewards, game_overs, w,
                                    float(discount), B, self.A, int(self.huber), 1.0, dq, self.A, td_errors,
                                    None, self.A, self.loss, self.status, ctx.stream)
-            self._backward_from_q(acts, q, saved, B)
-        self._apply_update(grad_scale, sync)
+            hold = False
+        ctx.hold_reductions = self.image and sync is None and not self.clip_gradients
+        try:
+            if hold:
+                self.torso.backward(ctx, acts)
+            else:
+                self._backward_from_q(acts, q, saved, B)
+        finally:
+            ctx.hold_reductions = False
+        try:
+            self._apply_update(grad_scale, sync)
+        except BaseException:
+            ctx.take_held()
+            raise
         return self.loss
 
 
diff --git a/include/rlx.h b/include/rlx.h
--- a/include/rlx.h
+++ b/include/rlx.h
@@ -447,6 +447,13 @@
                       float beta1, float beta2, float epsilon, float *state, float grad_scale, float *norm_out,
                       float *workspace, long long workspace_floats, const float *acc_src, float *acc_dst, int n_acc,
                       float *target, double mix_rate, unsigned int *ticket, void *stream);
+int rlx_adam_tf1_step_jobs_supported(const rlx_splitk_job *jobs_host, int n_jobs, const float *grads, long long n,
+                                     int with_norm, long long workspace_floats);
+int rlx_adam_tf1_step_jobs(const rlx_splitk_job *jobs_host, int n_jobs, float *weights, float *grads, float *m, float *v,
+                           long long n, float learning_rate, float beta1, float beta2, float epsilon, float *state,
+                           float grad_scale, float *norm_out, float *workspace, long long workspace_floats,
+                           const float *acc_src, float *acc_dst, int n_acc, float *target, double mix_rate,
+                           unsigned int *ticket, void *stream);
 int rlx_adam_norm_in_kernel(int on);
 int rlx_mix_weights(float *target, const float *online, long long n, double rate,
                     void *stream);
@@ -666,6 +673,8 @@
     float *workspace; long long workspace_floats;
 } rlx_conv_dw_item;
 int rlx_conv_dw_multi(const rlx_conv_dw_item *items_host, rlx_splitk_job *jobs_host, int n_items, void *stream);
+int rlx_conv_dw_multi_ppo_tail(const rlx_conv_dw_item *items_host, rlx_splitk_job *jobs_host, int n_items,
+                               const rlx_ppo_rows_desc *rows, void *stream);
 int rlx_conv_dw_passes(int passes);
 int rlx_conv_dw_pairs_per_workgroup(int pairs);
 
```

After: 38970 env-steps/s, median of 6. About the same (+0.9%).
